# CamilleChallier/Contrastive-Masked-UNet

Hardware: AMD Instinct MI355X
Metric: pretrain images/sec/node at 512x512 (CM-UNet masked-reconstruction step) (higher is better)
Workload: dtype f16; 1 GPU; cmunet_masked_recon_unet64x5_512x512_bs32_mask0.6; optimizer=AdamW(fused), amp=dynamic loss scale (device-side GradScaler protocol), global_batch=32, parallelism=dp1

## Files before the change

### cmunet_amd/_lib.py

```python
import ctypes
import os
import subprocess

_HERE = os.path.dirname(os.path.abspath(__file__))
CSRC = os.path.join(_HERE, "csrc")
LIB_PATH = os.environ.get("CMU_LIB_PATH") or os.path.join(CSRC, "libcmunet_hip.so")

F32, F16, BF16 = 0, 1, 2

_P = ctypes.c_void_p
_I = ctypes.c_int
_L = ctypes.c_int64
_F = ctypes.c_float
_U64 = ctypes.c_uint64
_D = ctypes.c_double

_SIGS = {
    "cmu_last_error": (ctypes.c_char_p, []),
    "cmu_last_kernel": (ctypes.c_char_p, []),
    "cmu_softmax2_threshold": (_I, [_P, _F, _P, _I, _I, _I, _P]),
    "cmu_conv3x3_c1_wgrad_bn": (_I, [_P, _P, _I, _P, _L, _P, _L, _P, _P, _P, _P, _P, _P, _I, _I, _I, _I, _I, _P, _P]),
    "cmu_conv3x3_c1_wgrad_bn_w": (_I, [_P, _P, _I, _P, _L, _P, _P, _P, _P, _P, _P, _P, _I, _I, _I, _I, _I, _P, _P]),
    "cmu_soft_skeleton_ws_bytes": (_L, [_L]),
    "cmu_soft_skeleton": (_I, [_P, _P, _I, _I, _I, _I, _P, _P]),
    "cmu_cldice_sums_ws_bytes": (_L, []),
    "cmu_cldice_sums": (_I, [_P, _P, _P, _P, _L, _P, _P, _P]),
    "cmu_softmax_planes": (_I, [_P, _P, _I, _I, _I, _F, _P, _P, _I, _I, _I, _I, _P]),
    "cmu_softmax_planes_bwd": (_I, [_P, _P, _I, _P, _I, _I, _I, _I, _P]),
    "cmu_soft_skeleton_save_ws_bytes": (_L, [_L, _I]),
    "cmu_soft_skeleton_save": (_I, [_P, _P, _I, _I, _I, _I, _P, _P]),
    "cmu_soft_skeleton_bwd_ws_bytes": (_L, [_L]),
    "cmu_soft_skeleton_bwd": (_I, [_P, _P, _P, _P, _P, _P, _P, _I, _I, _I, _I, _P, _P]),
    "cmu_argmax2_mask": (_I, [_P, _I, _P, _I, _I, _I, _I, _P]),
    "cmu_plane_mask": (_I, [_P, _I, _I, _I, _P, _I, _I, _I, _I, _P]),
    "cmu_contour_points_ws_bytes": (_L, [_I, _I, _I]),
    "cmu_contour_points": (_I, [_P, _P, _P, _I, _I, _I, _P, _P]),
    "cmu_lattice_nearest_ws_bytes": (_L, [_I, _I, _I]),
    "cmu_lattice_nearest": (_I, [_P, _P, _I, _P, _I, _I, _I, _P, _P]),
    "cmu_skeletonize": (_I, [_P, _P, _I, _I, _I, _P]),
    "cmu_hausdorff_finish": (_I, [_P, _P, _P, _P, _P, _P, _I, _P]),
    "cmu_radius_finish": (_I, [_P, _P, _P, _I, _P]),
    "cmu_sgd_step": (_I, [_P, _P, _P, _P, _L, _F, _F, _F, _F, _I, _L, _F, _P]),
    "cmu_sgd_step_amp": (_I, [_P, _P, _P, _P, _L, _F, _F, _F, _F, _I, _L, _F, _P, _P]),
    "cmu_lamb_block_elems": (_I, []),
    "cmu_lamb_ws_bytes": (_L, [_I, _I]),
    "cmu_resize_bicubic_ws_bytes": (_L, [_I, _I, _I, _I, _I]),
    "cmu_resize_bicubic": (_I, [_P, _I, _I, _I, _P, _P, _P, _I, _I, _P, _P]),
    "cmu_resize_bicubic_u8_ws_bytes": (_L, [_I, _I, _I, _I, _I]),
    "cmu_resize_bicubic_u8": (_I, [_P, _I, _I, _I, _P, _P, _P, _I, _I, _P, _P]),
    "cmu_resize_nearest_u8_ws_bytes": (_L, [_I, _I]),
    "cmu_resize_nearest_u8": (_I, [_P, _I, _I, _I, _P, _I, _I, _P, _P]),
    "cmu_two_view": (_I, [_P, _I, _I, _P, _P, _U64, _P, _P, _I, _P]),
    "cmu_philox_normal": (_I, [_P, _L, _U64, _U64, _P]),
    "cmu_random_patch_mask": (_I, [_P, _I, _I, _I, _I, _I, _U64, _U64, _P]),
    "cmu_skinny_gemm_ws_bytes": (_L, [_I, _I, _L]),
    "cmu_skinny_gemm_fwd": (_I, [_P, _P, _P, _P, _I, _I, _L, _P, _P]),
    "cmu_skinny_gemm_bwd_ws_bytes": (_L, [_I, _I]),
    "cmu_skinny_gemm_dgrad": (_I, [_P, _P, _P, _I, _I, _L, _P, _P]),
    "cmu_skinny_gemm_wgrad": (_I, [_P, _P, _P, _P, _I, _I, _L, _P]),
    "cmu_lamb_step": (_I, [_P, _P, _P, _P, _P, _P, _P, _P, _I, _P, _P, _I, _F, _F, _F, _F, _I, _I, _F, _I, _I, _L, _F, _P, _P]),
    "cmu_pack_desc_bytes": (_I, []),
    "cmu_pack_desc_blocks": (_L, [_I, _I, _I, _I, _I]),
    "cmu_pack_batch": (_I, [_P, _I, _L, _I, _P]),
    "cmu_version": (_I, []),
    "cmu_set_dispatch_override": (_I, [ctypes.c_char_p, _I]),
    "cmu_dispatch_knob_name": (ctypes.c_char_p, [_I]),
    "cmu_get_dispatch_knob": (_I, [ctypes.c_char_p, ctypes.POINTER(_I), ctypes.POINTER(_I)]),
    "cmu_mfma_sustained_rate": (_I, [_I, _I, _I, _I, _P, _P, _P, _P]),
    "cmu_probe_stream_reduce": (_I, [_P, _P, _P, _L, _I, _I, _P]),
    "cmu_dtype_size": (_I, [_I]),
    "cmu_pack_conv3x3_elems": (_L, [_I, _I, _I, _I]),
    "cmu_pack_conv3x3": (_I, [_P, _P, _I, _I, _I, _I, _P]),
    "cmu_pack_convT2x2_elems": (_L, [_I, _I, _I, _I]),
    "cmu_pack_convT2x2": (_I, [_P, _P, _I, _I, _I, _I, _P]),
    "cmu_conv3x3_c1_fwd": (_I, [_P, _P, _I, _P, _P, _L, _P, _I, _I, _I, _I, _I, _P]),
    "cmu_conv3x3_fwd": (_I, [_P, _L, _P, _P, _I, _P, _P, _L, _P, _I, _I, _I, _I, _I, _I, _P]),
    "cmu_conv_ntiles": (_I, [_I, _I, _I]),
    "cmu_bn_finalize_ws_bytes": (_L, [_I]),
    "cmu_bn_finalize": (_I, [_P, _I, _L, _P, _P, _P, _P, _P, _F, _F, _I, _P, _P, _P, _P, _I, _P, _P]),
    "cmu_bnrelu_maxpool_fwd": (_I, [_P, _L, _P, _P, _P, _L, _I, _I, _I, _I, _I, _P]),
    "cmu_convT2x2_fwd": (_I, [_P, _L, _P, _P, _I, _P, _P, _P, _L, _I, _I, _I, _I, _I, _I, _P]),
    "cmu_conv1x1_head_fwd": (_I, [_P, _L, _P, _P, _P, _P, _P, _I, _I, _I, _I, _I, _I, _P]),
    "cmu_apply_to_nchw": (_I, [_P, _L, _P, _P, _I, _P, _I, _I, _I, _I, _I, _P]),
    "cmu_nchw_to_nhwc": (_I, [_P, _P, _L, _I, _I, _I, _I, _I, _P]),
    "cmu_nhwc_to_nchw": (_I, [_P, _L, _P, _I, _I, _I, _I, _I, _P]),
    "cmu_bn_bwd_ws_bytes": (_L, [_I]),
    "cmu_bn_bwd_reduce": (_I, [_P, _L, _P, _L, _P, _P, _P, _P, _P, _P, _P, _I, _I, _I, _I, _I, _P, _P]),
    "cmu_bn_bwd_apply": (_I, [_P, _L, _P, _L, _P, _P, _P, _P, _P, _P, _L, _I, _I, _I, _I, _I, _P]),
    "cmu_conv3x3_wgrad_ws_bytes": (_L, [_I, _I, _I, _I, _I, _I]),
    "cmu_conv3x3_wgrad": (_I, [_P, _L, _P, _P, _I, _P, _L, _P, _I, _I, _I, _I, _I, _I, _P, _P]),
    "cmu_conv3x3_c1_wgrad_ws_bytes": (_L, [_I, _I, _I, _I]),
    "cmu_conv3x3_c1_wgrad": (_I, [_P, _P, _I, _P, _L, _P, _I, _I, _I, _I, _I, _P, _P]),
    "cmu_maxpool_bwd": (_I, [_P, _L, _P, _L, _P, _L, _P, _P, _P, _L, _P, _P, _P, _I, _I, _I, _I, _I, _P]),
    "cmu_maxpool_bwd2": (_I, [_P, _L, _P, _L, _P, _L, _P, _L, _P, _P, _P, _L, _P, _P, _P, _I, _I, _I, _I, _I, _P]),
    "cmu_maxpool_bwd_apply": (_I, [_P, _L, _P, _L, _P, _L, _P, _L, _P, _P, _P, _P, _P, _P, _L, _I, _I, _I, _I, _I, _P]),
    "cmu_bnrelu_maxpool_fwd_masked": (_I, [_P, _L, _P, _P, _P, _I, _P, _L, _I, _I, _I, _I, _I, _P]),
    "cmu_maxpool_bwd_masked": (_I, [_P, _L, _P, _L, _P, _L, _P, _P, _P, _I, _P, _L, _I, _I, _I, _I, _I, _P]),
    "cmu_bn_bwd_finalize": (_I, [_P, _L, _P, _P, _P, _I, _P]),
    "cmu_convT2x2_dgrad": (_I, [_P, _L, _P, _P, _L, _I, _I, _I, _I, _I, _I, _P]),
    "cmu_convT2x2_dgrad_bn": (_I, [_P, _L, _P, _P, _L, _P, _L, _P, _P, _P, _P, _P, _I, _I, _I, _I, _I, _I, _P]),
    "cmu_conv3x3_dgrad_bn": (_I, [_P, _L, _P, _P, _L, _P, _L, _P, _P, _P, _P, _P, _I, _I, _I, _I, _I, _I, _P]),
    "cmu_bn_bwd_finalize_tiles": (_I, [_P, _I, _L, _P, _P, _P, _I, _P, _P]),
    "cmu_convT2x2_wgrad_ws_bytes": (_L, [_I, _I, _I, _I, _I, _I]),
    "cmu_convT2x2_wgrad": (_I, [_P, _L, _P, _P, _I, _P, _L, _P, _P, _I, _I, _I, _I, _I, _I, _P, _P]),
    "cmu_conv1x1_head_bwd_ws_bytes": (_L, [_I, _I, _I, _I, _I]),
    "cmu_conv1x1_head_bn_apply": (_I, [_P, _P, _L, _P, _P, _P, _P, _P, _P, _P, _L, _I, _I, _I, _I, _I, _I, _P]),
    "cmu_conv1x1_head_bwd": (_I, [_P, _P, _L, _P, _P, _P, _P, _L, _P, _P, _P, _P, _P, _I, _I, _I, _I, _I, _I, _P, _P]),
    "cmu_masked_mse_ws_bytes": (_L, [_I, _I]),
    "cmu_masked_mse_fwd_bwd": (_I, [_P, _I, _I, _P, _P, _P, _P, _F, _P, _I, _I, _I, _P, _P]),
    "cmu_softmax_ce_dice_ws_bytes": (_L, [_I, _I, _I]),
    "cmu_softmax_ce_dice_fwd_bwd": (_I, [_P, _P, _P, _P, _F, _I, _I, _I, _P, _P]),
    "cmu_seg_stats_ws_bytes": (_L, [_I]),
    "cmu_seg_stats_fwd": (_I, [_P, _P, _I, _P, _F, _P, _I, _I, _I, _I, _P, _P]),
    "cmu_seg_stats_bwd": (_I, [_P, _P, _I, _P, _P, _P, _P, _P, _I, _I, _I, _I, _P]),
    "cmu_pointwise_loss_ws_bytes": (_L, []),
    "cmu_pointwise_loss_fwd": (_I, [_I, _P, _P, _I, _P, _P, _P, _L, _I, _L, _P, _P]),
    "cmu_pointwise_loss_bwd": (_I, [_I, _P, _P, _I, _P, _P, _P, _P, _L, _I, _L, _P]),
    "cmu_index_ce_ws_bytes": (_L, []),
    "cmu_index_ce_fwd": (_I, [_P, _P, _I, _I, _I, _P, _L, _P, _I, _I, _I, _I, _P, _P]),
    "cmu_index_ce_bwd": (_I, [_P, _P, _I, _I, _I, _P, _L, _P, _P, _I, _I, _I, _I, _P]),
    "cmu_infonce_inbatch_fwd_bwd": (_I, [_P, _P, _P, _P, _I, _I, _I, _I, _F, _F, _P]),
    "cmu_moco_ws_bytes": (_L, [_I, _I, _I]),
    "cmu_moco_infonce_enqueue": (_I, [_P, _P, _P, _I, _P, _P, _P, _P, _P, _I, _I, _I, _F, _P, _P]),
    "cmu_l2_normalize_rows": (_I, [_P, _P, _I, _I, _P]),
    "cmu_l2_normalize_rows_bwd": (_I, [_P, _P, _P, _I, _I, _P]),
    "cmu_moco_logits_assemble": (_I, [_P, _P, _P, _P, _I, _I, _I, _F, _P]),
    "cmu_moco_logits_split": (_I, [_P, _P, _I, _I, _F, _P]),
    "cmu_moco_logits_addpos": (_I, [_P, _P, _P, _I, _I, _I, _F, _P]),
    "cmu_row_cross_entropy": (_I, [_P, _P, _P, _P, _P, _P, _I, _I, _P]),
    "cmu_scale_by_device_scalar": (_I, [_P, _P, _L, _P]),
    "cmu_patchify": (_I, [_P, _P, _I, _I, _I, _I, _I, _I, _P]),
    "cmu_masked_stats_rows": (_I, []),
    "cmu_masked_channel_stats": (_I, [_P, _L, _P, _I, _I, _P, _I, _I, _I, _I, _I, _P]),
    "cmu_mask_select": (_I, [_P, _L, _P, _P, _I, _P, _I, _I, _P, _P, _L, _I, _I, _I, _I, _I, _P]),
    "cmu_bn_bwd_reduce_masked": (_I, [_P, _L, _P, _L, _P, _P, _P, _P, _P, _P, _P, _P, _I, _L, _I, _I, _I, _I, _I, _P, _P]),
    "cmu_bn_bwd_apply_masked": (_I, [_P, _L, _P, _L, _P, _P, _P, _P, _P, _P, _L, _P, _I, _I, _I, _I, _I, _I, _P]),
    "cmu_sparse_tile_list": (_I, [_P, _I, _I, _I, _I, _I, _I, _P, _P, _P]),
    "cmu_conv3x3_tiles_supported": (_I, [_I, _I, _I, _I, _I, _I]),
    "cmu_rows_channel_stats": (_I, [_P, _L, _P, _P, _P, _I, _I, _I, _I, _I, _P]),
    "cmu_bn_bwd_reduce_rows": (_I, [_P, _L, _P, _L, _P, _P, _P, _P, _P, _P, _P, _P, _P, _L, _L, _I, _I, _I, _I, _I, _P, _P]),
    "cmu_sparse_tile_lists_max": (_I, []),
    "cmu_sparse_tile_lists": (_I, [_P, _I, _I, _I, _P, _P, _P, _P, _P, _P]),
    "cmu_sparse_pixel_lists": (_I, [_P, _P, _I, _I, _I, _P, _P, _P, _P, _P]),
    "cmu_conv3x3_c1_fwd_tiles_rows": (_I, [_L]),
    "cmu_conv3x3_c1_fwd_tiles": (_I, [_P, _P, _I, _P, _P, _L, _P, _P, _P, _L, _I, _I, _I, _I, _I, _P]),
    "cmu_conv3x3_c1_wgrad_bn_tiles": (_I, [_P, _P, _I, _P, _L, _P, _L, _P, _P, _P, _P, _P, _P, _P, _P, _L, _P, _I, _I, _I, _I, _I, _P, _P]),
    "cmu_cells_supported": (_I, [_I, _I, _I, _I, _I, _I]),
    "cmu_bn_bwd_apply_cells": (_I, [_P, _L, _P, _L, _P, _P, _P, _P, _P, _P, _L, _P, _I, _I, _I, _I, _I, _I, _I, _P]),
    "cmu_mask_select_cells": (_I, [_P, _L, _P, _P, _I, _P, _I, _I, _P, _P, _L, _I, _I, _I, _I, _I, _P]),
    "cmu_maxpool_bwd_cells": (_I, [_P, _L, _P, _L, _P, _L, _P, _P, _P, _I, _P, _L, _I, _I, _I, _I, _I, _P]),
    "cmu_cells_stats_rows": (_I, []),
    "cmu_cells_channel_stats": (_I, [_P, _L, _P, _I, _P, _I, _I, _I, _I, _I, _P]),
    "cmu_bn_bwd_reduce_cells": (_I, [_P, _L, _P, _L, _P, _P, _P, _P, _P, _P, _P, _P, _I, _L, _I, _I, _I, _I, _I, _P, _P]),
    "cmu_cells_channel_sum_ws_bytes": (_L, [_I]),
    "cmu_cells_channel_sum": (_I, [_P, _L, _P, _I, _I, _P, _P, _I, _I, _I, _I, _I, _P]),
    "cmu_sparse_pixel_list_ws_bytes": (_L, [_I, _I]),
    "cmu_sparse_pixel_list": (_I, [_P, _I, _I, _I, _I, _P, _L, _P, _P, _P]),
    "cmu_conv3x3_rows_supported": (_I, [_I, _I, _I, _I, _I, _I]),
    "cmu_conv3x3_fwd_rows": (_I, [_P, _L, _P, _P, _L, _P, _P, _L, _I, _I, _I, _I, _I, _I, _P]),
    "cmu_conv3x3_fwd_tiles": (_I, [_P, _L, _P, _P, _I, _P, _P, _L, _P, _P, _I, _I, _I, _I, _I, _I, _P]),
    "cmu_conv3x3_wgrad_tile_h": (_I, [_I, _I, _I, _I, _I, _I]),
    "cmu_conv3x3_wgrad_tiles": (_I, [_P, _L, _P, _P, _I, _P, _L, _P, _P, _P, _I, _I, _I, _I, _I, _I, _I, _P, _P]),
    "cmu_spark_loss_ws_bytes": (_L, [_I, _I]),
    "cmu_spark_loss_fwd_bwd": (_I, [_P, _P, _P, _P, _P, _F, _I, _I, _I, _P, _P]),
    "cmu_gap_fwd": (_I, [_P, _L, _P, _P, _P, _I, _I, _I, _I, _I, _P]),
    "cmu_gap_bwd": (_I, [_P, _P, _L, _I, _I, _I, _I, _I, _P]),
    "cmu_ema_update": (_I, [_P, _P, _L, _F, _P]),
    "cmu_adam_step": (_I, [_P, _P, _P, _P, _P, _L, _F, _F, _F, _F, _F, _I, _L, _F, _P, _P]),
    "cmu_adam_ema_step": (_I, [_P, _P, _P, _P, _P, _L, _F, _F, _F, _F, _F, _I, _L, _F, _P, _I, _P, _P, _P, _F, _P]),
    "cmu_skinny16_gemm_ws_bytes": (_L, [_I, _I, _L]),
    "cmu_skinny16_gemm_fwd": (_I, [_P, _P, _P, _P, _I, _I, _L, _I, _P, _P]),
    "cmu_skinny16_gemm_dgrad": (_I, [_P, _P, _P, _I, _I, _L, _I, _P]),
    "cmu_skinny16_gemm_wgrad": (_I, [_P, _P, _P, _P, _I, _I, _L, _I, _P]),
    "cmu_bn1d_colsums": (_I, [_P, _P, _I, _I, _P]),
    "cmu_bn1d_relu_fwd": (_I, [_P, _P, _L, _P, _P, _P, _P, _F, _F, _I, _I, _P, _P, _P, _I, _I, _P]),
    "cmu_bn1d_bwd_colsums": (_I, [_P, _P, _P, _P, _P, _I, _P, _I, _I, _P]),
    "cmu_bn1d_relu_bwd": (_I, [_P, _P, _P, _P, _P, _P, _I, _P, _L, _P, _P, _P, _I, _I, _P]),
    "cmu_conv1x1_nchw_fwd": (_I, [_P, _L, _P, _P, _I, _P, _P, _P, _I, _I, _I, _I, _I, _I, _P]),
    "cmu_genesis_rec_bytes": (_I, []),
    "cmu_genesis_segments": (_I, [_I, _I]),
    "cmu_genesis_sample": (_I, [_P, _P, _P, _I, _I, _I, _I, _I, _D, _D, _D, _D, _D, _U64, _U64, _P]),
    "cmu_genesis_gather_shuffle": (_I, [_P, _P, _P, _P, _P, _P, _P, _I, _I, _I, _P]),
    "cmu_genesis_bezier_ws_bytes": (_L, [_I]),
    "cmu_genesis_bezier": (_I, [_P, _P, _I, _I, _I, _P, _P, _P]),
    "cmu_genesis_intensity_paint": (_I, [_P, _P, _P, _U64, _U64, _P, _I, _I, _I, _P]),
    "cmu_genesis_mae": (_I, [_P, _P, _P, _P, _P, _I, _I, _I, _P]),
    "cmu_ftaug_rec_layout": (_I, [_P, _I]),
    "cmu_ftaug_max_ksize": (_I, []),
    "cmu_ftaug_sample": (_I, [_P, _I, _I, _I, _I, _P, _I, _U64, _U64, _P]),
    "cmu_ftaug_photometric": (_I, [_P, _I, _I, _I, _P, _P, _U64, _U64, _I, _P, _I, _P]),
    "cmu_ftaug_apply": (_I, [_P, _P, _I, _I, _I, _P, _P, _U64, _U64, _I, _P, _P, _I, _P]),
    "cmu_ftaug_resize_ws_bytes": (_L, [_I, _I, _I]),
    "cmu_ftaug_resize_onehot": (_I, [_P, _P, _I, _I, _I, _P, _P, _U64, _U64, _I, _P, _I, _P, _P, _I, _I, _P, _P]),
    "cmu_mocoviews_rec_layout": (_I, [_P, _I]),
    "cmu_mocoviews_max_ksize": (_I, []),
    "cmu_mocoviews_sample": (_I, [_P, _I, _I, _I, _P, _I, _U64, _U64, _P]),
    "cmu_mocoviews_geometry": (_I, [_P, _I, _I, _I, _P, _I, _I, _I, _P, _I, _P, _P]),
    "cmu_mocoviews_max": (_I, [_P, _P, _I, _P]),
    "cmu_mocoviews_noise": (_I, [_P, _I, _I, _P, _P, _P, _U64, _U64, _P]),
    "cmu_mse_ws_bytes": (_L, []),
    "cmu_mse_fwd_bwd": (_I, [_P, _I, _P, _P, _P, _F, _P, _I, _I, _I, _P, _P]),
    "cmu_amp_state_bytes": (_I, []),
    "cmu_amp_init": (_I, [_P, _F, _P]),
    "cmu_amp_check_finite": (_I, [_P, _L, _P, _P]),
    "cmu_amp_update": (_I, [_P, _F, _F, _I, _P]),
}

EXPORTS = tuple(_SIGS.keys())


class CmuError(RuntimeError):
    pass


def build(verbose=False):
    jobs = str(min(8, os.cpu_count() or 1))
    res = subprocess.run(["make", "-C", CSRC, "-j", jobs], capture_output=not verbose, text=True)
    if res.returncode != 0:
        raise CmuError("building libcmunet_hip.so failed:\n" + (res.stdout or "") + (res.stderr or ""))
    return LIB_PATH


_lib = None


def lib():
    global _lib
    if _lib is None:
        if not os.path.exists(LIB_PATH):
            raise CmuError(f"{LIB_PATH} is missing: run `python -c 'import __graft_entry__ as g; g.build()'` "
                           "(hipcc --offload-arch=gfx950). The HIP path has no CPU fallback.")
        import torch
        l = ctypes.CDLL(LIB_PATH)
        for name, (res, args) in _SIGS.items():
            fn = getattr(l, name, None)
            if fn is None:
                continue
            fn.restype = res
            fn.argtypes = args
        _lib = l
    return _lib


def missing_symbols():
    l = lib()
    return [n for n in _SIGS if getattr(l, n, None) is None]


class EventProfiler:

    def __init__(self, gemm_only=False):
        self.records = []
        self.gemm_only = gemm_only

    def summary(self):
        import torch
        torch.cuda.synchronize()
        out = {}
        for name, e0, e1, work, _ in self.records:
            d = out.setdefault(name, {"ms": 0.0, "calls": 0, "work": 0.0})
            d["ms"] += e0.elapsed_time(e1)
            d["calls"] += 1
            d["work"] += work
        return out

    def by_kernel(self):
        import torch
        torch.cuda.synchronize()
        out = {}
        for name, e0, e1, work, tag in self.records:
            if work <= 0 or not tag:
                continue
            d = out.setdefault(tag, {"ms": 0.0, "calls": 0, "work": 0.0, "entries": set()})
            d["ms"] += e0.elapsed_time(e1)
            d["calls"] += 1
            d["work"] += work
            d["entries"].add(name)
        return out


PROFILER = None


class DevPtr(ctypes.c_void_p):
    """A device pointer that remembers which GPU owns it (``dev``): ``call`` binds the launch to that device."""


class _StreamOfArgs:
    """Placeholder for "the current stream of the device that owns this call's tensors" (resolved inside ``call``)."""


STREAM = _StreamOfArgs()


def devptr(addr, dev):
    p = DevPtr(addr)
    p.dev = dev
    return p


def call(name, *args, work=0.0):
    l = lib()
    fn = getattr(l, name, None)
    if fn is None:
        raise CmuError(f"{name} is not exported by {LIB_PATH}")
    import torch
    dev, si = None, -1
    for i, a in enumerate(args):
        if type(a) is DevPtr:
            if dev is None:
                dev = a.dev
            elif a.dev != dev:
                raise CmuError(f"{name}: tensors on different devices (cuda:{dev} and cuda:{a.dev})")
        elif a is STREAM:
            si = i
    cur = torch.cuda.current_device()
    if dev is None:
        dev = cur
    if si >= 0:
        args = list(args)
        args[si] = ctypes.c_void_p(torch.cuda.current_stream(dev).cuda_stream)
    if dev != cur:
        with torch.cuda.device(dev):
            return _call_bound(l, fn, name, args, work)
    return _call_bound(l, fn, name, args, work)


def _call_bound(l, fn, name, args, work):
    if PROFILER is not None and (work > 0 or not PROFILER.gemm_only):
        import torch
        e0, e1 = torch.cuda.Event(enable_timing=True), torch.cuda.Event(enable_timing=True)
        e0.record()
        rc = fn(*args)
        e1.record()
        PROFILER.records.append((name, e0, e1, work, l.cmu_last_kernel().decode() if work > 0 else ""))
    else:
        rc = fn(*args)
    if rc != 0:
        raise CmuError(f"{name} failed ({rc}): {l.cmu_last_error().decode()}")
    return rc
```

### cmunet_amd/csrc/conv_igemm.hip

```cpp
#include "common.h"
#include <stdlib.h>

enum { MODE_CONV3 = 0, MODE_CONVT_FWD = 1, MODE_CONVT_DGRAD = 2 };

struct IGParams {
    const void* x;
    int64_t ldx;
    const float* in_scale;
    const float* in_shift;
    int relu_from;
    const void* w;
    int npad;
    void* y;
    int64_t ldy;
    float* stats;
    const float* bias;
    int B, H, W;
    int K;
    int N;
    int Cq;
    int nslices;
    int nslices32;
    int tilesX, tilesY, nblk;
    int64_t total_blocks;
    const void* bx;
    int64_t ldbx;
    const float *b_scale, *b_shift, *b_mean, *b_invstd;
    float* bstats;
    int buf_ok;
    unsigned fd_nblk[2], fd_tx[2], fd_ty[2];
    const int* tile_list;
    const int* tile_count;
};
static inline void cmu_fastdiv_init(unsigned d, unsigned* out) {
    unsigned s = 0;
    while ((1ull << s) < d) ++s;
    out[0] = (unsigned)((((1ull << s) - d) << 32) / d + 1);
    out[1] = s;
}

template <class TR, int MODE>
struct IGCfg {
    typedef typename TR::elem_t elem_t;
    static constexpr bool C3 = (MODE == MODE_CONV3);
    static constexpr int TAPS = C3 ? 9 : 2;
    static constexpr int HALO = C3 ? 1 : 0;
    static constexpr int LW = CMU_TW + 2 * HALO;
    static constexpr int LH = CMU_TH + 2 * HALO;
    static constexpr int NPIX = LW * LH;
    static constexpr int SLICES_A = C3 ? 1 : TAPS;
    static constexpr int PS_A = SLICES_A * 64 + 16;
    static constexpr int A_BYTES = NPIX * PS_A;
    static constexpr int PS_W = 80;
    static constexpr int BN = 64;
    static constexpr int W_BYTES = TAPS * BN * PS_W;
    static constexpr int KC = 64 / (int)sizeof(elem_t);
    static constexpr int EPC = TR::EPC;
    static constexpr int EPI_ROW = BN * (int)sizeof(elem_t) + 16;
    static constexpr int EPI_STAGE = 4 * 64 * EPI_ROW;
    static constexpr int EPI_BYTES = EPI_STAGE + 4 * BN * 2 * 4;
    static constexpr int MAIN_BYTES = A_BYTES + W_BYTES;
    static constexpr int LDS_BYTES = MAIN_BYTES > EPI_BYTES ? MAIN_BYTES : EPI_BYTES;
    static constexpr int A_CHUNKS = NPIX * SLICES_A * 4;
    static constexpr int A_ITERS = (A_CHUNKS + 255) / 256;
    static constexpr int W_CHUNKS = TAPS * BN * 4;
    static constexpr int W_ITERS = (W_CHUNKS + 255) / 256;
};

__device__ static inline int pm_row(int r) { return __builtin_popcount(r >> 2) & 1; }
__device__ static inline int pm_col(int r) { return 4 * (r >> 3) + (r & 3); }

#ifdef CMU_IG_STAMPS
__device__ unsigned long long g_ig_stamps[64 * 16 * 8];
extern "C" int cmu_debug_ig_stamps(unsigned long long* host) {
    return (int)hipMemcpyFromSymbol(host, HIP_SYMBOL(g_ig_stamps), sizeof(g_ig_stamps));
}
#define IG_STAMP(k)                                                                          \
    do {                                                                                      \
        if (stamp_slot >= 0 && s < 16 && tid == 0)                                            \
            g_ig_stamps[(stamp_slot * 16 + s) * 8 + (k)] = __builtin_amdgcn_s_memtime();      \
    } while (0)
#else
#define IG_STAMP(k) do {} while (0)
#endif

template <class TR, int MODE>
__global__ __launch_bounds__(256, 2) void conv_igemm_kernel(const IGParams p) {
    typedef IGCfg<TR, MODE> C;
    typedef typename TR::elem_t elem_t;
    extern __shared__ __attribute__((aligned(16))) unsigned char smem[];

    const int tid = threadIdx.x;
    const int lane = tid & 63;
    const int wave = tid >> 6;
    const int r = lane & 31;
    const int h = lane >> 5;

    int64_t bid = blockIdx.x;
    {
        const int64_t nb = p.total_blocks;
        const int64_t q = nb >> 3, rem = nb & 7;
        const int64_t xcd = bid & 7, local = bid >> 3;
        bid = (xcd < rem ? xcd * (q + 1) : rem * (q + 1) + (xcd - rem) * q) + local;
    }
    const int nbk = (int)(bid % p.nblk);
    const int64_t tile = bid / p.nblk;
    const int tx = (int)(tile % p.tilesX);
    const int ty = (int)((tile / p.tilesX) % p.tilesY);
    const int b = (int)(tile / ((int64_t)p.tilesX * p.tilesY));
    const int ty0 = ty * CMU_TH, tx0 = tx * CMU_TW;
    const int n0 = nbk * C::BN;

    const int Hin = (MODE == MODE_CONVT_DGRAD) ? 2 * p.H : p.H;
    const int Win = (MODE == MODE_CONVT_DGRAD) ? 2 * p.W : p.W;
    const unsigned char* xb = reinterpret_cast<const unsigned char*>(p.x);
// ... 164 lines not shown
#pragma unroll
        for (int it = 0; it < C::W_ITERS; ++it) {
            if (it * 256 + tid < C::W_CHUNKS) *reinterpret_cast<u32x4*>(smem + w_lds[it]) = wreg[it];
        }
    };

    f32x16 acc[2][2];
#pragma unroll
    for (int i = 0; i < 2; ++i)
#pragma unroll
        for (int j = 0; j < 2; ++j)
#pragma unroll
            for (int e = 0; e < 16; ++e) acc[i][j][e] = 0.f;

    int a_base[2];
#pragma unroll
    for (int i = 0; i < 2; ++i) a_base[i] = ((4 * wave + 2 * i + pm_row(r)) * C::LW + pm_col(r)) * C::PS_A + h * 16;
    const int w_base = C::A_BYTES + r * C::PS_W + h * 16;

    const int nstages = C::C3 ? p.nslices : (p.nslices + C::TAPS - 1) / C::TAPS;

#ifdef CMU_IG_STAMPS
    const int stamp_slot = (blockIdx.x % 61 == 0 && blockIdx.x / 61 < 64) ? (int)(blockIdx.x / 61) : -1;
#endif
    load_stage(0);
    for (int s = 0; s < nstages; ++s) {
        IG_STAMP(0);
        __syncthreads();
        IG_STAMP(1);
        store_stage();
        IG_STAMP(2);
        __syncthreads();
        IG_STAMP(3);
        if (s + 1 < nstages) load_stage(s + 1);
        IG_STAMP(4);
#pragma unroll
        for (int t = 0; t < C::TAPS; ++t) {
            const int aoff = C::C3 ? ((t / 3) * C::LW + (t % 3)) * C::PS_A : t * 64;
#pragma unroll
            for (int ks = 0; ks < 2; ++ks) {
                const u32x4 a0 = *reinterpret_cast<const u32x4*>(smem + a_base[0] + aoff + ks * 32);
                const u32x4 a1 = *reinterpret_cast<const u32x4*>(smem + a_base[1] + aoff + ks * 32);
                const u32x4 b0 = *reinterpret_cast<const u32x4*>(smem + w_base + (t * C::BN) * C::PS_W + ks * 32);
                const u32x4 b1 = *reinterpret_cast<const u32x4*>(smem + w_base + (t * C::BN + 32) * C::PS_W + ks * 32);
                TR::mma16(a0, b0, acc[0][0]);
                TR::mma16(a0, b1, acc[0][1]);
                TR::mma16(a1, b0, acc[1][0]);
                TR::mma16(a1, b1, acc[1][1]);
            }
        }
        IG_STAMP(5);
    }
    __syncthreads();

    float* stat_lds = reinterpret_cast<float*>(smem + C::EPI_STAGE);
    if (MODE == MODE_CONV3 && p.stats != nullptr) {
        float s1[2] = {0.f, 0.f}, s2[2] = {0.f, 0.f};
#pragma unroll
        for (int i = 0; i < 2; ++i)
#pragma unroll
            for (int e = 0; e < 16; ++e) {
                const int m32 = (e & 3) + 8 * (e >> 2) + 4 * h;
                const int row = 4 * wave + 2 * i + pm_row(m32), col = pm_col(m32);
                const bool ok = (ty0 + row < p.H) && (tx0 + col < p.W);
#pragma unroll
                for (int j = 0; j < 2; ++j) {
                    const float v = ok ? acc[i][j][e] : 0.f;
                    s1[j] += v;
                    s2[j] = fmaf(v, v, s2[j]);
                }
            }
#pragma unroll
        for (int j = 0; j < 2; ++j) {
            s1[j] += __shfl_xor(s1[j], 32, 64);
            s2[j] += __shfl_xor(s2[j], 32, 64);
            if (h == 0) {
                stat_lds[(wave * C::BN + 32 * j + r) * 2 + 0] = s1[j];
                stat_lds[(wave * C::BN + 32 * j + r) * 2 + 1] = s2[j];
            }
        }
    }
    constexpr int CPRp = C::BN / C::EPC;
    u32x4 xr[CPRp];
    if ((MODE != MODE_CONVT_FWD) && p.bstats != nullptr) {
#pragma unroll
        for (int it = 0; it < CPRp; ++it) {
            const int idx = it * 64 + lane;
            const int m = idx / CPRp, q = idx % CPRp;
            const int row = 4 * wave + 2 * (m >> 5) + pm_row(m & 31), col = pm_col(m & 31);
            const int gy = ty0 + row < p.H ? ty0 + row : p.H - 1, gx = tx0 + col < p.W ? tx0 + col : p.W - 1;
            int n = n0 + q * C::EPC;
            n = n < p.N ? n : 0;
            const int64_t xo = (((int64_t)b * p.H + gy) * p.W + gx) * p.ldbx + n;
            xr[it] = ld_global16(reinterpret_cast<const unsigned char*>(p.bx) + xo * (int64_t)sizeof(elem_t));
        }
    }
    unsigned char* my = smem + wave * (64 * C::EPI_ROW);
#pragma unroll
    for (int i = 0; i < 2; ++i)
#pragma unroll
        for (int j = 0; j < 2; ++j) {
            float badd = 0.f;
            if (MODE == MODE_CONVT_FWD) {
                const int n = n0 + 32 * j + r;
                if (n < p.N) badd = p.bias[n % p.Cq];
            }
#pragma unroll
            for (int e = 0; e < 16; ++e) {
                const int m = 32 * i + (e & 3) + 8 * (e >> 2) + 4 * h;
                *reinterpret_cast<elem_t*>(my + m * C::EPI_ROW + (32 * j + r) * (int)sizeof(elem_t)) =
                    TR::from_float(acc[i][j][e] + badd);
            }
        }
    __syncthreads();
    if (MODE == MODE_CONV3 && p.stats != nullptr && tid < C::BN) {
        const int n = n0 + tid;
        if (n < p.N) {
            float a = 0.f, q = 0.f;
#pragma unroll
            for (int w4 = 0; w4 < 4; ++w4) {
                a += stat_lds[(w4 * C::BN + tid) * 2 + 0];
                q += stat_lds[(w4 * C::BN + tid) * 2 + 1];
            }
            p.stats[(tile * 2 + 0) * p.N + n] = a;
            p.stats[(tile * 2 + 1) * p.N + n] = q;
        }
    }
    constexpr int CPR = C::BN / C::EPC;
    unsigned char* yb = reinterpret_cast<unsigned char*>(p.y);
    const bool bs = (MODE != MODE_CONVT_FWD) && p.bstats != nullptr;
    constexpr int EPCc = C::EPC;
    float bsc[EPCc], bsh[EPCc], bmu[EPCc], bis[EPCc], bs1[EPCc], bs2[EPCc];
    const int nq = n0 + (lane % CPR) * EPCc;
    if (bs) {
#pragma unroll
        for (int e = 0; e < EPCc; ++e) {
            const int c = nq + e < p.N ? nq + e : 0;
            bsc[e] = p.b_scale[c]; bsh[e] = p.b_shift[c]; bmu[e] = p.b_mean[c]; bis[e] = p.b_invstd[c];
            bs1[e] = bs2[e] = 0.f;
        }
    }
#pragma unroll
    for (int it = 0; it < (64 * CPR) / 64; ++it) {
        const int idx = it * 64 + lane;
        const int m = idx / CPR, q = idx % CPR;
        const int row = 4 * wave + 2 * (m >> 5) + pm_row(m & 31), col = pm_col(m & 31);
        const int gy = ty0 + row, gx = tx0 + col;
        const int n = n0 + q * C::EPC;
        if (gy < p.H && gx < p.W && n < p.N) {
            const u32x4 v = *reinterpret_cast<const u32x4*>(my + m * C::EPI_ROW + q * 16);
            int64_t off;
            if (MODE == MODE_CONVT_FWD) {
                const int ij = n / p.Cq, co = n % p.Cq;
                off = (((int64_t)b * (2 * p.H) + 2 * gy + (ij >> 1)) * (2 * p.W) + 2 * gx + (ij & 1)) * p.ldy + co;
            } else {
                off = (((int64_t)b * p.H + gy) * p.W + gx) * p.ldy + n;
            }
            st_global16(yb + off * (int64_t)sizeof(elem_t), v);
            if (bs) {
                float gv[EPCc], xv[EPCc];
                TR::unpack(v, gv);
                TR::unpack(xr[it], xv);
#pragma unroll
                for (int e = 0; e < EPCc; ++e) {
                    const float dz = fmaf(xv[e], bsc[e], bsh[e]) > 0.f ? gv[e] : 0.f;
                    bs1[e] += dz;
                    bs2[e] = fmaf(dz, xv[e], bs2[e]);
                }
            }
        }
    }
    if (bs) {
#pragma unroll
        for (int e = 0; e < EPCc; ++e) {
#pragma unroll
            for (int o = CPR; o < 64; o <<= 1) {
                bs1[e] += __shfl_xor(bs1[e], o, 64);
                bs2[e] += __shfl_xor(bs2[e], o, 64);
            }
            bs2[e] = (bs2[e] - bmu[e] * bs1[e]) * bis[e];
            if (lane < CPR) {
                stat_lds[(wave * C::BN + lane * EPCc + e) * 2 + 0] = bs1[e];
                stat_lds[(wave * C::BN + lane * EPCc + e) * 2 + 1] = bs2[e];
            }
        }
        __syncthreads();
        if (tid < C::BN && n0 + tid < p.N) {
            float a = 0.f, q = 0.f;
#pragma unroll
            for (int w4 = 0; w4 < 4; ++w4) {
                a += stat_lds[(w4 * C::BN + tid) * 2 + 0];
                q += stat_lds[(w4 * C::BN + tid) * 2 + 1];
            }
            p.bstats[(tile * 2 + 0) * p.N + n0 + tid] = a;
            p.bstats[(tile * 2 + 1) * p.N + n0 + tid] = q;
        }
    }
}

#include "conv_igemm3.inc"
#include "conv_igemm3p.inc"
#include "conv_igemm5.inc"
#include "conv_igemm6.inc"
#include "conv_gemm.inc"
#include "conv_gather.inc"

template <class TR, int MODE>
static int launch_igemm(const IGParams& p, hipStream_t st, const char* name) {
    typedef IGCfg<TR, MODE> C;
    static CmuPerDevice attr_set;
    if (!attr_set.done()) {
        hipError_t e = hipFuncSetAttribute(reinterpret_cast<const void*>(&conv_igemm_kernel<TR, MODE>),
                                           hipFuncAttributeMaxDynamicSharedMemorySize, C::LDS_BYTES);
        if (e != hipSuccess) {
            cmu_set_error("%s: hipFuncSetAttribute(%d B LDS): %s", name, C::LDS_BYTES, hipGetErrorString(e));
            return CMU_ERR_LAUNCH;
        }
        attr_set.mark();
    }
    hipLaunchKernelGGL((conv_igemm_kernel<TR, MODE>), dim3((unsigned)p.total_blocks), dim3(256), C::LDS_BYTES, st, p);
    cmu_set_kernel_tag("conv_igemm_kernel");
    CMU_CHECK_LAUNCH(name);
    return CMU_OK;
}

static int check_act(const char* name, const void* ptr, int64_t ld, int C, int dt) {
    const int epc = 16 / cmu_dtype_size(dt);
    CMU_CHECK_ARG(ptr != nullptr, "%s: null tensor", name);
    CMU_CHECK_ARG(cmu_aligned16(ptr), "%s: tensor not 16-byte aligned", name);
    CMU_CHECK_ARG(ld >= C && ld % epc == 0, "%s: pixel stride %lld must be >= C=%d and a multiple of %d", name, (long long)ld, C, epc);
    CMU_CHECK_ARG(C % epc == 0, "%s: channels %d must be a multiple of %d", name, C, epc);
    return CMU_OK;
}

template <class TR>
static int conv3x3_fwd_t(IGParams p, hipStream_t st) {
    typedef IGCfg<TR, MODE_CONV3> C;
    if (igemm3_eligible<TR>(p)) return launch_igemm3_any<TR>(p, st);
    p.nslices = cmu_div_up(p.K, C::KC);
    p.nslices32 = cmu_div_up(p.K, C::KC / 2);
    p.npad = cmu_conv3x3_npad(p.N);
    p.buf_ok = cmu_knob(CMU_KNOB_CONV_BUFLOAD) && ((int64_t)p.H * p.W * p.ldx + p.K) * (int64_t)sizeof(typename TR::elem_t) < 0x7fff0000ll &&
               (int64_t)p.nslices32 * 9 * p.npad * 32 < 0x7fff0000ll;
    return launch_igemm<TR, MODE_CONV3>(p, st, "cmu_conv3x3_fwd");
}
template <class TR>
static int convT_fwd_t(IGParams p, hipStream_t st) {
    typedef IGCfg<TR, MODE_CONVT_FWD> C;
    if (conv_gemm_s_eligible<TR>(p, false))
        return p.in_scale ? launch_conv_gemm_s<TR, false, true>(p, st, "cmu_convT2x2_fwd") : launch_conv_gemm_s<TR, false, false>(p, st, "cmu_convT2x2_fwd");
    if (conv_gemm_eligible<TR>(p, false))
        return p.in_scale ? launch_conv_gemm<TR, false, true>(p, st, "cmu_convT2x2_fwd") : launch_conv_gemm<TR, false, false>(p, st, "cmu_convT2x2_fwd");
    p.nslices = cmu_div_up(p.K, C::KC);
    return launch_igemm<TR, MODE_CONVT_FWD>(p, st, "cmu_convT2x2_fwd");
}
template <class TR>
static int convT_dgrad_t(IGParams p, hipStream_t st) {
    typedef IGCfg<TR, MODE_CONVT_DGRAD> C;
    {
        IGParams q = p;
        q.K = 4 * p.K;
        if (conv_gemm_s_eligible<TR>(q, true)) return launch_conv_gemm_s<TR, true, false>(q, st, "cmu_convT2x2_dgrad");
        if (conv_gemm_eligible<TR>(q, true)) return launch_conv_gemm<TR, true, false>(q, st, "cmu_convT2x2_dgrad");
    }
    p.nslices = 4 * cmu_div_up(p.K, C::KC);
    return launch_igemm<TR, MODE_CONVT_DGRAD>(p, st, "cmu_convT2x2_dgrad");
}

static void fill_tiles(IGParams& p) {
    p.tilesX = cmu_div_up(p.W, CMU_TW);
    p.tilesY = cmu_div_up(p.H, CMU_TH);
    p.nblk = cmu_div_up(p.N, 64);
    p.npad = p.nblk * 64;
    p.total_blocks = (int64_t)p.B * p.tilesX * p.tilesY * p.nblk;
}

extern "C" int cmu_conv_ntiles(int B, int H, int W) { return B * cmu_div_up(H, CMU_TH) * cmu_div_up(W, CMU_TW); }

// ... 257 lines not shown
    hipLaunchKernelGGL(sparse_tile_lists_kernel, dim3(n), dim3(1024), 0, (hipStream_t)stream, active, q);
    CMU_CHECK_LAUNCH("cmu_sparse_tile_lists");
    return CMU_OK;
}
struct SpRowsBatch {
    int f;
    int s[SP_MAX_LISTS], H[SP_MAX_LISTS];
    int* rows[SP_MAX_LISTS];
    int* count[SP_MAX_LISTS];
    long long cap[SP_MAX_LISTS];
};
__global__ void sparse_pixel_rows_multi_kernel(const int* __restrict__ plist, const int* __restrict__ pcount, SpRowsBatch q) {
    const int i = blockIdx.y;
    const int np = pcount[0], s = q.s[i], H = q.H[i], f = q.f;
    const long long n = (long long)np * s * s, cap = q.cap[i];
    int* __restrict__ rows = q.rows[i];
    for (long long r = (long long)blockIdx.x * blockDim.x + threadIdx.x; r < cap; r += (long long)gridDim.x * blockDim.x) {
        int v = -1;
        if (r < n) {
            const int pi = (int)(r / (s * s)), in = (int)(r % (s * s));
            const int t = plist[pi];
            const int fx = t % f, fy = (t / f) % f, b = t / (f * f);
            v = (b * H + fy * s + in / s) * H + fx * s + in % s;
        }
        rows[r] = v;
    }
    if (blockIdx.x == 0 && threadIdx.x == 0) q.count[i][0] = (int)(n < cap ? n : cap);
}
extern "C" int cmu_sparse_pixel_lists(const int* patches, const int* patch_count, int f, int B, int n, const int* H, int* const* rows,
                                      const int64_t* capacity, int* const* counts, void* stream) {
    CMU_CHECK_ARG(patches && patch_count && f > 0 && B > 0 && n > 0 && n <= SP_MAX_LISTS && H && rows && capacity && counts,
                  "cmu_sparse_pixel_lists: bad args (at most %d levels per call)", SP_MAX_LISTS);
    SpRowsBatch q = {};
    q.f = f;
    int64_t cmax = 0;
    for (int i = 0; i < n; ++i) {
        const int sb = sp_shift_bits(H[i], f);
        CMU_CHECK_ARG(rows[i] && counts[i] && capacity[i] > 0 && sb >= 0 && (int64_t)B * H[i] * H[i] < (1ll << 31),
                      "cmu_sparse_pixel_lists: null list, or H must be f << s (entry %d: H=%d, f=%d)", i, H[i], f);
        q.s[i] = 1 << sb; q.H[i] = H[i]; q.rows[i] = rows[i]; q.count[i] = counts[i]; q.cap[i] = capacity[i];
        if (capacity[i] > cmax) cmax = capacity[i];
    }
    const int grid = (int)(cmu_div_up64(cmax, 256) < 4096 ? cmu_div_up64(cmax, 256) : 4096);
    hipLaunchKernelGGL(sparse_pixel_rows_multi_kernel, dim3(grid, n), dim3(256), 0, (hipStream_t)stream, patches, patch_count, q);
    CMU_CHECK_LAUNCH("cmu_sparse_pixel_lists");
    return CMU_OK;
}
extern "C" int cmu_sparse_tile_list(const uint8_t* active, int f, int B, int H, int W, int tile_h, int tile_w, int* list, int* count,
                                    void* stream) {
    CMU_CHECK_ARG(active && list && count && f > 0 && B > 0 && H > 0 && W > 0 && tile_h > 0 && tile_w > 0, "cmu_sparse_tile_list: bad args");
    const int sbits = sp_shift_bits(H, f);
    CMU_CHECK_ARG(sbits >= 0 && W == H, "cmu_sparse_tile_list: H must be f << s and the level square (H=%d, W=%d, f=%d)", H, W, f);
    const int tilesY = cmu_div_up(H, tile_h), tilesX = cmu_div_up(W, tile_w);
    CMU_CHECK_ARG((int64_t)B * tilesY * tilesX < (1ll << 30), "cmu_sparse_tile_list: too many tiles");
    hipLaunchKernelGGL(sparse_tile_list_kernel, dim3(1), dim3(1024), 0, (hipStream_t)stream, active, f, sbits, B, tilesY, tilesX, tile_h, tile_w,
                       list, count);
    CMU_CHECK_LAUNCH("cmu_sparse_tile_list");
    return CMU_OK;
}

static int check_bnstats(const char* name, const void* yraw, int64_t ldy, const float* scale, const float* shift, const float* mean,
                         const float* invstd, const float* bstats, int N, int dt) {
    int rc;
    if ((rc = check_act(name, yraw, ldy, N, dt))) return rc;
    CMU_CHECK_ARG(scale && shift && mean && invstd && bstats, "%s: null BatchNorm argument", name);
    return CMU_OK;
}

extern "C" int cmu_conv3x3_dgrad_bn(const void* dY, int64_t ldd, const void* wpacked_flip, void* dX, int64_t ldx, const void* yraw,
                                    int64_t ldy, const float* scale, const float* shift, const float* save_mean,
                                    const float* save_invstd, float* bstats, int B, int H, int W, int K, int N, int dt, void* stream) {
    CMU_CHECK_ARG(B > 0 && H > 0 && W > 0 && K > 0 && N > 0, "cmu_conv3x3_dgrad_bn: bad dims");
    CMU_CHECK_ARG(cmu_dtype_size(dt) > 0, "cmu_conv3x3_dgrad_bn: bad dtype %d", dt);
    int rc;
    if ((rc = check_act("cmu_conv3x3_dgrad_bn(dY)", dY, ldd, K, dt))) return rc;
    if ((rc = check_act("cmu_conv3x3_dgrad_bn(dX)", dX, ldx, N, dt))) return rc;
    if ((rc = check_bnstats("cmu_conv3x3_dgrad_bn(yraw)", yraw, ldy, scale, shift, save_mean, save_invstd, bstats, N, dt))) return rc;
    CMU_CHECK_ARG(wpacked_flip && cmu_aligned16(wpacked_flip), "cmu_conv3x3_dgrad_bn: packed weights null/unaligned");
    CMU_CHECK_ARG((int64_t)B * cmu_div_up(H, CMU_TH) * cmu_div_up(W, CMU_TW) * cmu_div_up(N, 64) < (1ll << 31), "cmu_conv3x3_dgrad_bn: grid too large");
    IGParams p = {};
    p.x = dY; p.ldx = ldd; p.w = wpacked_flip; p.y = dX; p.ldy = ldx;
    p.B = B; p.H = H; p.W = W; p.K = K; p.N = N; p.Cq = N;
    p.bx = yraw; p.ldbx = ldy; p.b_scale = scale; p.b_shift = shift; p.b_mean = save_mean; p.b_invstd = save_invstd; p.bstats = bstats;
    fill_tiles(p);
    CMU_DISPATCH_DT(dt, conv3x3_fwd_t, p, (hipStream_t)stream);
}

extern "C" int cmu_convT2x2_dgrad_bn(const void* dOut, int64_t ldd, const void* wpacked_dgrad, void* dX, int64_t ldx, const void* yraw,
                                     int64_t ldy, const float* scale, const float* shift, const float* save_mean,
                                     const float* save_invstd, float* bstats, int B, int H, int W, int Cin, int Cout, int dt,
                                     void* stream) {
    CMU_CHECK_ARG(B > 0 && H > 0 && W > 0 && Cin > 0 && Cout > 0, "cmu_convT2x2_dgrad_bn: bad dims");
    CMU_CHECK_ARG(cmu_dtype_size(dt) > 0, "cmu_convT2x2_dgrad_bn: bad dtype %d", dt);
    int rc;
    if ((rc = check_act("cmu_convT2x2_dgrad_bn(dOut)", dOut, ldd, Cout, dt))) return rc;
    if ((rc = check_act("cmu_convT2x2_dgrad_bn(dX)", dX, ldx, Cin, dt))) return rc;
    if ((rc = check_bnstats("cmu_convT2x2_dgrad_bn(yraw)", yraw, ldy, scale, shift, save_mean, save_invstd, bstats, Cin, dt))) return rc;
    CMU_CHECK_ARG(wpacked_dgrad && cmu_aligned16(wpacked_dgrad), "cmu_convT2x2_dgrad_bn: packed weights null/unaligned");
    IGParams p = {};
    p.x = dOut; p.ldx = ldd; p.w = wpacked_dgrad; p.y = dX; p.ldy = ldx;
    p.B = B; p.H = H; p.W = W; p.K = Cout; p.N = Cin; p.Cq = Cout;
    p.bx = yraw; p.ldbx = ldy; p.b_scale = scale; p.b_shift = shift; p.b_mean = save_mean; p.b_invstd = save_invstd; p.bstats = bstats;
    fill_tiles(p);
    CMU_DISPATCH_DT(dt, convT_dgrad_t, p, (hipStream_t)stream);
}
```

### cmunet_amd/csrc/conv_igemm3.inc

```
#include <type_traits>

template <class TR, int NB_, int TWB_ = 2, int THB_ = 1>
struct IG3Cfg {
    typedef typename TR::elem_t elem_t;
    static constexpr int ES = (int)sizeof(elem_t);
    static constexpr int EPC = TR::EPC;
    static constexpr int KC = 32 / ES;
    static constexpr int NB = NB_;
    static constexpr int TWB = TWB_;
    static constexpr int THB = THB_;
    static constexpr int TH = 16 * THB, TW = 16 * TWB;
    static constexpr int LW = TW + 2, LH = TH + 2, NPIX = LW * LH;
    static constexpr int PS = 48;
    static constexpr int A_BYTES = NPIX * PS;
    static constexpr int PSB = 32;
    static constexpr int B_TAP = NB * PSB;
    static constexpr int B_BYTES = 9 * B_TAP;
    static constexpr int BUF_BYTES = A_BYTES + B_BYTES;
    static constexpr int MAIN_BYTES = 2 * BUF_BYTES;
    static constexpr int WN = NB / 64, WM = 8 / WN;
    static constexpr int RB = WM / TWB;
    static constexpr int SW = TH / 2 / RB;
    static constexpr int A_CHUNKS = NPIX * 2, A_ITERS = (A_CHUNKS + 511) / 512;
    static constexpr int B_CHUNKS = 9 * NB * 2, B_ITERS = (B_CHUNKS + 511) / 512;
    static constexpr int MAX_K = THB == 1 ? 1024 : 128;
    static constexpr int TAB_BYTES = 2 * MAX_K * 4;
    static constexpr int NFP = ES == 2 ? 2 : 1;
    static constexpr int EPI_ROW = NFP * 32 * ES + 16;
    static constexpr int EPI_WAVE = SW * 32 * EPI_ROW;
    static constexpr int EPI_STAGE = 8 * EPI_WAVE;
    static constexpr int EPI_BYTES = EPI_STAGE + 8 * 64 * 2 * 4;
#ifdef CMU_IG_STAMPS
    static constexpr int STAMP_OFF = MAIN_BYTES + TAB_BYTES;
    static constexpr int LDS_BYTES = (STAMP_OFF + 2048 > EPI_BYTES ? STAMP_OFF + 2048 : EPI_BYTES);
#else
    static constexpr int LDS_BYTES = MAIN_BYTES + TAB_BYTES > EPI_BYTES ? MAIN_BYTES + TAB_BYTES : EPI_BYTES;
#endif
    static constexpr unsigned OOB = 0x7fff0000u;
};

__device__ static inline u32x4 ig3_bload(__amdgpu_buffer_rsrc_t r, unsigned voff, unsigned soff) {
    return __builtin_bit_cast(u32x4, __builtin_amdgcn_raw_buffer_load_b128(r, (int)voff, (int)soff, 0));
}

typedef __attribute__((ext_vector_type(2))) float f32x2;
template <int SW, class OK>
__device__ __forceinline__ void ig3_lane_stats(const f32x16 (&acc)[SW][2], OK ok, float (&s1)[2], float (&s2)[2]) {
    f32x2 a[2], q[2];
#pragma unroll
    for (int j = 0; j < 2; ++j) a[j] = q[j] = f32x2{0.f, 0.f};
#pragma unroll
    for (int i = 0; i < SW; ++i)
#pragma unroll
        for (int e = 0; e < 16; e += 2) {
            const bool ok0 = ok(i, e), ok1 = ok(i, e + 1);
#pragma unroll
            for (int j = 0; j < 2; ++j) {
                const f32x2 v = {ok0 ? acc[i][j][e] : 0.f, ok1 ? acc[i][j][e + 1] : 0.f};
                a[j] += v;
                q[j] = __builtin_elementwise_fma(v, v, q[j]);
            }
        }
#pragma unroll
    for (int j = 0; j < 2; ++j) {
        s1[j] = a[j][0] + a[j][1];
        s2[j] = q[j][0] + q[j][1];
    }
}

template <int EPC>
__device__ __forceinline__ void ig3_bst_consts(const float* scale, const float* shift, int n, float (&gs)[EPC], float (&gh)[EPC]) {
#pragma unroll
    for (int e = 0; e < EPC; ++e) {
        gs[e] = scale[n + e] * 0x1p60f;
        gh[e] = shift[n + e] * 0x1p60f;
    }
}
template <class TR>
__device__ __forceinline__ void ig3_bst_accum(const u32x4& g, const u32x4& x, const float (&gs)[TR::EPC], const float (&gh)[TR::EPC],
                                              float (&bs1)[TR::EPC], float (&bs2)[TR::EPC]) {
    float gv[TR::EPC], xv[TR::EPC];
    TR::unpack(g, gv);
    TR::unpack(x, xv);
#pragma unroll
    for (int e = 0; e < TR::EPC; e += 2) {
        const float gate0 = __builtin_amdgcn_fmed3f(fmaf(xv[e], gs[e], gh[e]), 0.f, 1.f);
        const float gate1 = __builtin_amdgcn_fmed3f(fmaf(xv[e + 1], gs[e + 1], gh[e + 1]), 0.f, 1.f);
        const f32x2 dz = f32x2{gate0, gate1} * f32x2{gv[e], gv[e + 1]};
        const f32x2 s1 = f32x2{bs1[e], bs1[e + 1]} + dz;
        const f32x2 s2 = __builtin_elementwise_fma(dz, f32x2{xv[e], xv[e + 1]}, f32x2{bs2[e], bs2[e + 1]});
        bs1[e] = s1[0]; bs1[e + 1] = s1[1];
        bs2[e] = s2[0]; bs2[e + 1] = s2[1];
    }
}
template <int EPC>
__device__ __forceinline__ void ig3_bst_fold(float (&bs1)[EPC], float (&bs2)[EPC], int lane, const float* mean, const float* invstd, float* stat) {
    constexpr int H1 = EPC / 2, H2 = EPC / 4;
    float a1[H1], a2[H1], b1[H2], b2[H2];
    auto fold32 = [](float d, float s) {
        const auto r = __builtin_amdgcn_permlane32_swap(__float_as_uint(d), __float_as_uint(s), false, false);
        return __uint_as_float(r[0]) + __uint_as_float(r[1]);
    };
    auto fold16 = [](float d, float s) {
        const auto r = __builtin_amdgcn_permlane16_swap(__float_as_uint(d), __float_as_uint(s), false, false);
        return __uint_as_float(r[0]) + __uint_as_float(r[1]);
    };
    auto fold8 = [](float v) { return v + __uint_as_float(__builtin_amdgcn_update_dpp(0u, __float_as_uint(v), 0x128 , 0xf, 0xf, false)); };
#pragma unroll
    for (int e = 0; e < H1; ++e) { a1[e] = fold32(bs1[e], bs1[e + H1]); a2[e] = fold32(bs2[e], bs2[e + H1]); }
#pragma unroll
    for (int e = 0; e < H2; ++e) { b1[e] = fold8(fold16(a1[e], a1[e + H2])); b2[e] = fold8(fold16(a2[e], a2[e + H2])); }
    const int c0 = (lane & 7) * EPC + H1 * (lane >> 5) + H2 * ((lane >> 4) & 1);
    if (!(lane & 8)) {
#pragma unroll
        for (int e = 0; e < H2; ++e) {
            stat[(c0 + e) * 2 + 0] = b1[e];
            stat[(c0 + e) * 2 + 1] = (b2[e] - mean[c0 + e] * b1[e]) * invstd[c0 + e];
        }
    }
}

template <class TR, int NB, int TWB>
__device__ __forceinline__ void ig3_epilogue(const IGParams& p, unsigned char* smem, f32x16 (&acc)[IG3Cfg<TR, NB, TWB>::SW][2], int tid, int lane,
                                             int wave, int wn, int wrow, int wcol, int r, int h, int b, int ty, int tx, int ty0, int tx0,
                                             int n0) {
    typedef IG3Cfg<TR, NB, TWB> C;
    typedef typename TR::elem_t elem_t;
    constexpr int EPC = TR::EPC;
    constexpr int SW = C::SW;
    float* stat_lds = reinterpret_cast<float*>(smem + C::EPI_STAGE);
    const int row0 = wrow * 2 * SW, col0 = wcol * 16;
    if (p.stats != nullptr) {
        float s1[2], s2[2];
        ig3_lane_stats<SW>(acc, [&](int i, int e) {
            const int m32 = (e & 3) + 8 * (e >> 2) + 4 * h;
            const int row = row0 + 2 * i + pm_row(m32), col = col0 + pm_col(m32);
            return (ty0 + row < p.H) && (tx0 + col < p.W);
        }, s1, s2);
#pragma unroll
        for (int j = 0; j < 2; ++j) {
            s1[j] += __shfl_xor(s1[j], 32, 64);
            s2[j] += __shfl_xor(s2[j], 32, 64);
            if (h == 0) {
                stat_lds[(wave * 64 + 32 * j + r) * 2 + 0] = s1[j];
                stat_lds[(wave * 64 + 32 * j + r) * 2 + 1] = s2[j];
            }
        }
    }
    unsigned char* my = smem + wave * C::EPI_WAVE;
    unsigned char* yb = reinterpret_cast<unsigned char*>(p.y);
    constexpr int CPR = C::NFP * 32 / EPC;
    auto write_slab = [&](float* dst) {
        if (tid < TWB * NB) {
            const int half = tid / NB, c = tid % NB;
            const int tx16 = TWB * tx + half, tiles16 = (p.W + 15) / 16;
            if (tx16 < tiles16 && n0 + c < p.N) {
                float a = 0.f, q = 0.f;
#pragma unroll
                for (int wr = 0; wr < C::RB; ++wr) {
                    const int wv = (c / 64) * C::WM + wr * TWB + half;
                    a += stat_lds[(wv * 64 + (c & 63)) * 2 + 0];
                    q += stat_lds[(wv * 64 + (c & 63)) * 2 + 1];
                }
                const int64_t t16 = ((int64_t)b * p.tilesY + ty) * tiles16 + tx16;
                dst[(t16 * 2 + 0) * p.N + n0 + c] = a;
                dst[(t16 * 2 + 1) * p.N + n0 + c] = q;
            }
        }
    };
    constexpr int NIT = (SW * 32 * CPR) / 64;
    float badd[2] = {0.f, 0.f};
    const bool cq64 = p.bias != nullptr && (p.Cq & 63) == 0;
    int ij_w = 0, co_w = 0;
    if (p.bias != nullptr) {
        const int nw = n0 + wn * 64;
        ij_w = nw / p.Cq;
        co_w = nw - ij_w * p.Cq;
#pragma unroll
        for (int j = 0; j < 2; ++j) badd[j] = p.bias[cq64 ? co_w + 32 * j + r : (nw + 32 * j + r) % p.Cq];
    }
#pragma unroll
    for (int jp = 0; jp < 2 / C::NFP; ++jp) {
        if (jp > 0) __syncthreads();
        u32x4 xr[NIT];
        if (p.bstats != nullptr) {
#pragma unroll
            for (int it = 0; it < NIT; ++it) {
                const int idx = it * 64 + lane;
                const int m = idx / CPR, q = idx % CPR;
                const int row = row0 + 2 * (m >> 5) + pm_row(m & 31), col = col0 + pm_col(m & 31);
                const int gy = ty0 + row < p.H ? ty0 + row : p.H - 1, gx = tx0 + col < p.W ? tx0 + col : p.W - 1;
                const int n = n0 + wn * 64 + jp * C::NFP * 32 + q * EPC;
                const int64_t pixel = ((int64_t)b * p.H + gy) * p.W + gx;
                xr[it] = ld_global16(reinterpret_cast<const unsigned char*>(p.bx) + (pixel * p.ldbx + n) * (int64_t)sizeof(elem_t));
            }
        }
#pragma unroll
        for (int i = 0; i < SW; ++i)
#pragma unroll
            for (int jj = 0; jj < C::NFP; ++jj)
#pragma unroll
                for (int e = 0; e < 16; ++e) {
                    const int m = 32 * i + (e & 3) + 8 * (e >> 2) + 4 * h;
                    *reinterpret_cast<elem_t*>(my + m * C::EPI_ROW + (32 * jj + r) * C::ES) =
                        TR::from_float(acc[i][jp * C::NFP + jj][e] + badd[jp * C::NFP + jj]);
                }
        __syncthreads();
        if (jp == 0 && p.stats != nullptr) write_slab(p.stats);
        float bsc[EPC], bsh[EPC], bs1[EPC], bs2[EPC];
        const int nq = n0 + wn * 64 + jp * C::NFP * 32 + (lane % CPR) * EPC;
        if (p.bstats != nullptr) {
            ig3_bst_consts<EPC>(p.b_scale, p.b_shift, nq, bsc, bsh);
#pragma unroll
            for (int e = 0; e < EPC; ++e) bs1[e] = bs2[e] = 0.f;
        }
#pragma unroll
        for (int it = 0; it < NIT; ++it) {
            const int idx = it * 64 + lane;
            const int m = idx / CPR, q = idx % CPR;
            const int row = row0 + 2 * (m >> 5) + pm_row(m & 31), col = col0 + pm_col(m & 31);
            const int gy = ty0 + row, gx = tx0 + col;
            const int n = n0 + wn * 64 + jp * C::NFP * 32 + q * EPC;
            if (gy < p.H && gx < p.W) {
                const u32x4 v = *reinterpret_cast<const u32x4*>(my + m * C::EPI_ROW + q * 16);
                const int64_t pixel = ((int64_t)b * p.H + gy) * p.W + gx;
                if (p.bias != nullptr) {
                    const int ij = cq64 ? ij_w : n / p.Cq, co = cq64 ? co_w + (n - (n0 + wn * 64)) : n % p.Cq;
                    const int64_t po = ((int64_t)b * (2 * p.H) + 2 * gy + (ij >> 1)) * (2 * p.W) + 2 * gx + (ij & 1);
                    st_global16_nt(yb + (po * p.ldy + co) * (int64_t)sizeof(elem_t), v);
                } else {
                    st_global16_nt(yb + (pixel * p.ldy + n) * (int64_t)sizeof(elem_t), v);
                }
                if (p.bstats != nullptr) ig3_bst_accum<TR>(v, xr[it], bsc, bsh, bs1, bs2);
            }
        }
        if (p.bstats != nullptr) {
            const int nb0 = n0 + wn * 64 + jp * C::NFP * 32;
            ig3_bst_fold<EPC>(bs1, bs2, lane, p.b_mean + nb0, p.b_invstd + nb0, stat_lds + (wave * 64 + jp * C::NFP * 32) * 2);
        }
    }
    if (p.bstats != nullptr) {
        __syncthreads();
        write_slab(p.bstats);
    }
}

template <class TR, int NB, bool TF, int TWB>
__global__ __launch_bounds__(512) void conv_igemm3_kernel(const IGParams p) {
    typedef IG3Cfg<TR, NB, TWB> C;
    constexpr int EPC = TR::EPC;
    constexpr int SW = C::SW;
    extern __shared__ __attribute__((aligned(16))) unsigned char smem[];

    const int tid = threadIdx.x;
    const int lane = tid & 63;
    const int wave = __builtin_amdgcn_readfirstlane(tid >> 6);
    const int r = lane & 31;
    const int h = lane >> 5;
    const int wm = wave % C::WM, wn = wave / C::WM;
    const int wcol = wm % TWB, wrow = wm / TWB;

    int64_t bid = blockIdx.x;
    {
        const int64_t nb = p.total_blocks;
        const int64_t q = nb >> 3, rem = nb & 7;
        const int64_t xcd = bid & 7, local = bid >> 3;
        bid = (xcd < rem ? xcd * (q + 1) : rem * (q + 1) + (xcd - rem) * q) + local;
    }
    const int nbk = (int)(bid % p.nblk);
    const int64_t tile = bid / p.nblk;
    const int tx = (int)(tile % p.tilesX);
    const int ty = (int)((tile / p.tilesX) % p.tilesY);
    const int b = (int)(tile / ((int64_t)p.tilesX * p.tilesY));
    const int ty0 = ty * C::TH, tx0 = tx * C::TW;
    const int n0 = nbk * NB;

    const int64_t img_elems = (int64_t)p.H * p.W * p.ldx;
    const unsigned char* ximg = reinterpret_cast<const unsigned char*>(p.x) + (int64_t)b * img_elems * C::ES;
    const unsigned x_bytes = (unsigned)((((int64_t)p.H * p.W - 1) * p.ldx + p.K) * C::ES);
    const __amdgpu_buffer_rsrc_t rs_x = __builtin_amdgcn_make_buffer_rsrc(const_cast<unsigned char*>(ximg), 0, (int)x_bytes, 0x00020000);
    const unsigned w_bytes = (unsigned)((int64_t)p.nslices32 * 9 * p.npad * 32);
    const __amdgpu_buffer_rsrc_t rs_w = __builtin_amdgcn_make_buffer_rsrc(const_cast<void*>(p.w), 0, (int)w_bytes, 0x00020000);

    const int cg = tid & 1;
    unsigned a_voff[C::A_ITERS];
    unsigned a_inb = 0;
#pragma unroll
    for (int it = 0; it < C::A_ITERS; ++it) {
        const int pix = it * 256 + (tid >> 1);
        const int py = pix / C::LW, px = pix % C::LW;
        const int gy = ty0 - 1 + py, gx = tx0 - 1 + px;
        const bool ok = pix < C::NPIX && gy >= 0 && gy < p.H && gx >= 0 && gx < p.W;
        a_voff[it] = ok ? (unsigned)((((int64_t)gy * p.W + gx) * p.ldx + cg * EPC) * C::ES) : C::OOB;
        a_inb |= (ok ? 1u : 0u) << it;
    }
    const bool a_last_live = ((C::A_ITERS - 1) * 256 + (tid >> 1)) < C::NPIX;
    const unsigned a_st = (unsigned)((tid >> 1) * C::PS + cg * 16);
    unsigned b_voff[C::B_ITERS];
#pragma unroll
    for (int it = 0; it < C::B_ITERS; ++it) {
        const int row = it * 256 + (tid >> 1);
        const int t = row / NB, n = row % NB;
        b_voff[it] = row < 9 * NB ? (unsigned)(((int64_t)t * p.npad + n0 + n) * 32 + cg * 16) : C::OOB;
    }
    const bool b_last_live = ((C::B_ITERS - 1) * 256 + (tid >> 1)) < 9 * NB;
    const unsigned b_st = (unsigned)(C::A_BYTES + (tid >> 1) * C::PSB + ((cg ^ ((tid >> 4) & 1)) * 16));
    const unsigned w_slice = (unsigned)p.npad * 32u * 9u;

    u32x4 areg[C::A_ITERS], breg[C::B_ITERS];
    const int nsl = p.nslices32;
    float* tab = reinterpret_cast<float*>(smem + C::MAIN_BYTES);
    if (TF)
        for (int c = tid; c < p.K; c += 512) {
            tab[c] = p.in_scale[c];
            tab[C::MAX_K + c] = p.in_shift[c];
        }
    auto issue_loads = [&](int s) {
#pragma unroll
        for (int it = 0; it < C::A_ITERS; ++it) areg[it] = ig3_bload(rs_x, a_voff[it], (unsigned)(s * 32));
#pragma unroll
        for (int it = 0; it < C::B_ITERS; ++it) breg[it] = ig3_bload(rs_w, b_voff[it], (unsigned)s * w_slice);
    };
    auto store_regs = [&](unsigned buf, int s) {
        float sc[EPC], sh[EPC];
        float lo = 0.f;
        if (TF) {
// ... 221 lines not shown
```

### cmunet_amd/csrc/conv_igemm3p.inc

```

template <class TR, int NB, int THB = 1, bool WRES = false>
struct IG3PCfg {
    typedef IG3Cfg<TR, NB, 2, THB> C;
    static constexpr int WRES_SLICES = 4;
    static constexpr int A_STRIDE = WRES ? C::A_BYTES : C::BUF_BYTES;
    static constexpr int B_BASE = WRES ? 2 * C::A_BYTES : C::A_BYTES;
    static constexpr int MAIN_BYTES = WRES ? 2 * C::A_BYTES + WRES_SLICES * C::B_BYTES : C::MAIN_BYTES;
    static constexpr int STAT_OFF = MAIN_BYTES + C::TAB_BYTES;
    static constexpr int STAT_BYTES = 8 * 64 * 2 * 4;
    static constexpr int EPI_OFF = STAT_OFF + STAT_BYTES;
    static constexpr int EPI_WAVE1 = 16 * C::EPI_ROW;
#ifdef CMU_IG_STAMPS
    static constexpr int STAMP_OFF = MAIN_BYTES + 1024;
    static constexpr int STAMP_ITERS = 12;
    static constexpr int LDS_BYTES = EPI_OFF + 8 * EPI_WAVE1;
#else
    static constexpr int LDS_BYTES = EPI_OFF + 8 * EPI_WAVE1;
#endif
};

template <class TR, int NB, bool TF, bool BST, int THB = 1, bool WRES = false, bool PART = false>
__global__ __launch_bounds__(512) void conv_igemm3p_kernel(const IGParams p) {
    typedef IG3Cfg<TR, NB, 2, THB> C;
    typedef IG3PCfg<TR, NB, THB, WRES> P;
// ... 483 lines not shown
            s_regs = s_ld;
            inb_regs = a_inb;
        }
#ifndef CMU_IG_STAMPS_EPI
        IG3P_STAMP(5);
#endif
        if (++s_mma == nsl) {
            s_mma = 0;
            ++i_mma;
        }
        if (!second) __syncthreads();
#ifndef CMU_IG_STAMPS_EPI
        IG3P_STAMP(6);
#endif
    }
    __syncthreads();
#ifdef CMU_IG_STAMPS
    if (stamp_slot >= 0 && tid < 2 * P::STAMP_ITERS * 8) g_ig_stamps[stamp_slot * 256 + tid] = stamp_lds[tid];
    if (stamp_slot >= 0 && tid == 0) {
        g_ig_stamps[stamp_slot * 256 + 200] = __builtin_amdgcn_s_memtime() - clk0;
        g_ig_stamps[stamp_slot * 256 + 201] = __builtin_amdgcn_s_memrealtime() - rt0;
        g_ig_stamps[stamp_slot * 256 + 202] = (unsigned long long)G;
    }
#endif
    write_slab(decode(n_my - 1));
}

static int cmu_num_cus() {
    static int n[256] = {0};
    const int dev = cmu_current_device() & 255;
    int v = __atomic_load_n(&n[dev], __ATOMIC_RELAXED);
    if (v == 0) {
        int cus = 0;
        if (hipDeviceGetAttribute(&cus, hipDeviceAttributeMultiprocessorCount, dev) != hipSuccess || cus <= 0) cus = 256;
        v = cus;
        __atomic_store_n(&n[dev], v, __ATOMIC_RELAXED);
    }
    return v;
}

template <class TR, int NB, bool TF, bool BST, int THB = 1, bool WRES = false, bool PART = false>
static int launch_igemm3p_cfg(IGParams p, hipStream_t st) {
    typedef IG3Cfg<TR, NB, 2, THB> C;
    typedef IG3PCfg<TR, NB, THB, WRES> P;
    static_assert(P::LDS_BYTES <= 163840, "LDS budget");
    static CmuPerDevice attr_set;
    if (!attr_set.done()) {
        hipError_t e = hipFuncSetAttribute(reinterpret_cast<const void*>(&conv_igemm3p_kernel<TR, NB, TF, BST, THB, WRES, PART>),
                                           hipFuncAttributeMaxDynamicSharedMemorySize, P::LDS_BYTES);
        if (e != hipSuccess) {
            cmu_set_error("cmu_conv3x3_fwd(wide, persistent): hipFuncSetAttribute(%d B LDS): %s", P::LDS_BYTES, hipGetErrorString(e));
            return CMU_ERR_LAUNCH;
        }
        attr_set.mark();
    }
    p.tilesX = cmu_div_up(p.W, C::TW);
    p.tilesY = cmu_div_up(p.H, C::TH);
    p.nblk = p.N / NB;
    p.nslices32 = p.K / C::KC;
    p.nslices = p.nslices32;
    p.npad = cmu_conv3x3_npad(p.N);
    p.total_blocks = (int64_t)p.B * p.tilesX * p.tilesY * p.nblk;
    if (p.total_blocks >= (1ll << 30)) return launch_igemm3_cfg<TR, NB, TF, 2>(p, st);
    cmu_fastdiv_init((unsigned)p.nblk, p.fd_nblk);
    cmu_fastdiv_init((unsigned)p.tilesX, p.fd_tx);
    cmu_fastdiv_init((unsigned)p.tilesY, p.fd_ty);
    const int forced = cmu_knob(CMU_KNOB_CONV_PERSIST_GRID);
    const int64_t want = forced > 0 ? forced : cmu_num_cus();
    const int64_t grid = p.total_blocks < want ? p.total_blocks : want;
    hipLaunchKernelGGL((conv_igemm3p_kernel<TR, NB, TF, BST, THB, WRES, PART>), dim3((unsigned)grid), dim3(512), P::LDS_BYTES, st, p);
    cmu_set_kernel_tag("conv_igemm3p_kernel");
    CMU_CHECK_LAUNCH("cmu_conv3x3_fwd(wide, persistent)");
    return CMU_OK;
}

static bool cmu_conv_persist_enabled() { return cmu_knob(CMU_KNOB_CONV_PERSIST); }
template <class TR> static bool igemm5_eligible(const IGParams& p);
template <class TR> static int launch_igemm5(const IGParams& p, hipStream_t st);
template <class TR> static bool igemm6_eligible(const IGParams& p);
template <class TR> static int launch_igemm6(const IGParams& p, hipStream_t st);
template <class TR>
static int launch_igemm3_any(const IGParams& p, hipStream_t st) {
    if (!cmu_conv_persist_enabled()) return launch_igemm3<TR>(p, st);
    if (igemm6_eligible<TR>(p)) return launch_igemm6<TR>(p, st);
    if (igemm5_eligible<TR>(p)) return launch_igemm5<TR>(p, st);
    const bool tf = p.in_scale != nullptr, bst = p.bstats != nullptr;
    if (tf && bst) return launch_igemm3<TR>(p, st);
    if (p.K / (32 / (int)sizeof(typename TR::elem_t)) < 4) return launch_igemm3<TR>(p, st);
    if (p.H % 16 != 0 || p.W % 32 != 0) {
        if (!igemm3_persist_part_enabled() || igemm3_slim_tiles(p, (int)sizeof(typename TR::elem_t))) return launch_igemm3<TR>(p, st);
        if (p.N % 128 == 0 && !igemm3_narrow_blocks(p))
            return tf ? launch_igemm3p_cfg<TR, 128, true, false, 1, false, true>(p, st)
                      : (bst ? launch_igemm3p_cfg<TR, 128, false, true, 1, false, true>(p, st) : launch_igemm3p_cfg<TR, 128, false, false, 1, false, true>(p, st));
        return tf ? launch_igemm3p_cfg<TR, 64, true, false, 1, false, true>(p, st)
                  : (bst ? launch_igemm3p_cfg<TR, 64, false, true, 1, false, true>(p, st) : launch_igemm3p_cfg<TR, 64, false, false, 1, false, true>(p, st));
    }
    if (p.N % 128 == 0 && !igemm3_narrow_blocks(p))
        return tf ? launch_igemm3p_cfg<TR, 128, true, false>(p, st)
                  : (bst ? launch_igemm3p_cfg<TR, 128, false, true>(p, st) : launch_igemm3p_cfg<TR, 128, false, false>(p, st));
    if constexpr (sizeof(typename TR::elem_t) == 2) {
        if (cmu_knob(CMU_KNOB_CONV_WRES) && p.N == 64 && p.K == 64)
            return tf ? launch_igemm3p_cfg<TR, 64, true, false, 1, true>(p, st)
                      : (bst ? launch_igemm3p_cfg<TR, 64, false, true, 1, true>(p, st) : launch_igemm3p_cfg<TR, 64, false, false, 1, true>(p, st));
    }
    return tf ? launch_igemm3p_cfg<TR, 64, true, false>(p, st)
              : (bst ? launch_igemm3p_cfg<TR, 64, false, true>(p, st) : launch_igemm3p_cfg<TR, 64, false, false>(p, st));
}
```

### cmunet_amd/csrc/elementwise.hip

```cpp
#include "common.h"
#include <string.h>

static thread_local char g_err[512] = "";
void cmu_set_error(const char* fmt, ...) {
    va_list ap;
    va_start(ap, fmt);
    vsnprintf(g_err, sizeof(g_err), fmt, ap);
    va_end(ap);
}
extern "C" const char* cmu_last_error(void) { return g_err; }
static thread_local const char* g_kernel_tag = "";
void cmu_set_kernel_tag(const char* tag) { g_kernel_tag = tag; }
extern "C" const char* cmu_last_kernel(void) { return g_kernel_tag; }
extern "C" int cmu_version(void) { return 100; }

#define CMU_KNOB_UNREAD INT32_MIN
struct CmuKnobRow {
    const char* name;
    int kind, dflt, floor;
    int env = CMU_KNOB_UNREAD, ovr = -1;
};
#define CMU_KNOB_ROW(id, kind, dflt, floor) {"CMU_" #id, CMU_KNOB_##kind, dflt, floor},
static CmuKnobRow g_knobs[CMU_KNOB_COUNT] = {CMU_KNOBS(CMU_KNOB_ROW)};
int cmu_knob(int id) {
// ... 527 lines not shown
    CMU_DISPATCH_DT(dt, conv3x3_c1_fwd_t, x, mask, mask_per_sample, w, y, ldy, stats, B, H, W, Cout, (hipStream_t)stream);
}

extern "C" int cmu_conv3x3_c1_fwd_tiles_rows(int64_t max_tiles) { return (int)(max_tiles < CMU_C1F_CAP ? (max_tiles < 1 ? 1 : max_tiles) : CMU_C1F_CAP); }
extern "C" int cmu_conv3x3_c1_fwd_tiles(const float* x, const uint8_t* mask, int mask_per_sample, const float* w, void* y, int64_t ldy,
                                        float* stats, const int* tile_list, const int* tile_count, int64_t max_tiles, int B, int H, int W,
                                        int Cout, int dt, void* stream) {
    const int es = cmu_dtype_size(dt);
    CMU_CHECK_ARG(es > 0, "cmu_conv3x3_c1_fwd_tiles: bad dtype");
    const int epc = 16 / es;
    CMU_CHECK_ARG(x && w && y && tile_list && tile_count && B > 0 && H > 0 && W > 0, "cmu_conv3x3_c1_fwd_tiles: bad args");
    CMU_CHECK_ARG(Cout % epc == 0 && Cout / epc <= 256 && Cout > 0, "cmu_conv3x3_c1_fwd_tiles: Cout=%d must be a multiple of %d (<= %d)", Cout, epc, 256 * epc);
    CMU_CHECK_ARG(cmu_aligned16(y) && ldy % epc == 0 && ldy >= Cout, "cmu_conv3x3_c1_fwd_tiles: y alignment / stride");
    if (max_tiles < 1) max_tiles = 1;
    CMU_DISPATCH_DT(dt, conv3x3_c1_fwd_t, x, mask, mask_per_sample, w, y, ldy, stats, B, H, W, Cout, (hipStream_t)stream, tile_list, tile_count,
                    max_tiles);
}

template <class TR>
__global__ void bnrelu_maxpool_kernel(const unsigned char* __restrict__ y, int64_t ldy, const float* __restrict__ scale,
                                      const float* __restrict__ shift, unsigned char* __restrict__ out, int64_t ldo, int B, int H,
                                      int W, int C, int64_t total, const uint8_t* __restrict__ amask = nullptr, int f = 0, int sbits = 0) {
    constexpr int EPC = TR::EPC;
    constexpr int ES = (int)sizeof(typename TR::elem_t);
    const int nchunk = C / EPC;
    const int Ho = H / 2, Wo = W / 2;
    for (int64_t o = (int64_t)blockIdx.x * blockDim.x + threadIdx.x; o < total; o += (int64_t)gridDim.x * blockDim.x) {
        int ch, xo, yo, b;
        int64_t pix;
        if (total <= 0x7fffffffll) {
            const unsigned ou = (unsigned)o, pq = ou / (unsigned)nchunk;
            ch = (int)(ou - pq * (unsigned)nchunk);
            pix = pq;
        } else {
            ch = (int)(o % nchunk);
            pix = o / nchunk;
        }
        cmu_pixel_coords(pix, Wo, Ho, total <= 0x7fffffffll, b, yo, xo);
        if (amask != nullptr && !sp_active(amask, f, sbits, b, 2 * yo, 2 * xo, 0)) {
            st_global16(out + ((((int64_t)b * Ho + yo) * Wo + xo) * ldo + ch * EPC) * ES, u32x4{0u, 0u, 0u, 0u});
            continue;
        }
        float sc[EPC], sh[EPC], m[EPC];
#pragma unroll
        for (int e = 0; e < EPC; ++e) {
            sc[e] = scale[ch * EPC + e];
            sh[e] = shift[ch * EPC + e];
            m[e] = 0.f;
        }
#pragma unroll
        for (int q = 0; q < 4; ++q) {
            const int64_t src = (((int64_t)b * H + 2 * yo + (q >> 1)) * W + 2 * xo + (q & 1)) * ldy + ch * EPC;
            float f[EPC];
            TR::unpack(ld_global16_nt(y + src * ES), f);
#pragma unroll
            for (int e = 0; e < EPC; ++e) m[e] = fmaxf(m[e], fmaf(f[e], sc[e], sh[e]));
        }
        st_global16(out + ((((int64_t)b * Ho + yo) * Wo + xo) * ldo + ch * EPC) * ES, TR::pack(m));
    }
}
template <class TR>
static int bnrelu_maxpool_t(const void* y, int64_t ldy, const float* scale, const float* shift, void* out, int64_t ldo, int B, int H,
                            int W, int C, hipStream_t st, const uint8_t* amask = nullptr, int f = 0) {
    const int64_t total = (int64_t)B * (H / 2) * (W / 2) * (C / TR::EPC);
#ifndef CMU_POOLF_CAP
#define CMU_POOLF_CAP 65536
#endif
    const int grid = (int)(cmu_div_up64(total, 256) < CMU_POOLF_CAP ? cmu_div_up64(total, 256) : CMU_POOLF_CAP);
    hipLaunchKernelGGL((bnrelu_maxpool_kernel<TR>), dim3(grid), dim3(256), 0, st, (const unsigned char*)y, ldy, scale, shift,
                       (unsigned char*)out, ldo, B, H, W, C, total, amask, f, amask ? sp_shift_bits(H, f) : 0);
    CMU_CHECK_LAUNCH("cmu_bnrelu_maxpool_fwd");
    return CMU_OK;
}
extern "C" int cmu_bnrelu_maxpool_fwd(const void* y, int64_t ldy, const float* scale, const float* shift, void* out, int64_t ldo,
                                      int B, int H, int W, int C, int dt, void* stream) {
    const int es = cmu_dtype_size(dt);
    CMU_CHECK_ARG(es > 0 && y && out && scale && shift, "cmu_bnrelu_maxpool_fwd: bad args");
    const int epc = 16 / es;
    CMU_CHECK_ARG(H % 2 == 0 && W % 2 == 0 && H > 0 && W > 0 && B > 0, "cmu_bnrelu_maxpool_fwd: H,W must be even (got %d,%d)", H, W);
    CMU_CHECK_ARG(C % epc == 0 && ldy % epc == 0 && ldo % epc == 0 && ldy >= C && ldo >= C, "cmu_bnrelu_maxpool_fwd: C/ld alignment");
    CMU_CHECK_ARG(cmu_aligned16(y) && cmu_aligned16(out), "cmu_bnrelu_maxpool_fwd: pointer alignment");
    CMU_DISPATCH_DT(dt, bnrelu_maxpool_t, y, ldy, scale, shift, out, ldo, B, H, W, C, (hipStream_t)stream);
}
extern "C" int cmu_bnrelu_maxpool_fwd_masked(const void* y, int64_t ldy, const float* scale, const float* shift, const uint8_t* active, int f,
                                             void* out, int64_t ldo, int B, int H, int W, int C, int dt, void* stream) {
    const int es = cmu_dtype_size(dt);
    CMU_CHECK_ARG(es > 0 && y && out && scale && shift && active && f > 0, "cmu_bnrelu_maxpool_fwd_masked: bad args");
    const int epc = 16 / es;
    CMU_CHECK_ARG(H % 2 == 0 && W % 2 == 0 && H > 0 && W > 0 && B > 0, "cmu_bnrelu_maxpool_fwd_masked: H,W must be even (got %d,%d)", H, W);
    CMU_CHECK_ARG(C % epc == 0 && ldy % epc == 0 && ldo % epc == 0 && ldy >= C && ldo >= C, "cmu_bnrelu_maxpool_fwd_masked: C/ld alignment");
    CMU_CHECK_ARG(cmu_aligned16(y) && cmu_aligned16(out), "cmu_bnrelu_maxpool_fwd_masked: pointer alignment");
    const int sbits = sp_shift_bits(H, f);
    CMU_CHECK_ARG(sbits >= 1 && (f << sbits) == W, "cmu_bnrelu_maxpool_fwd_masked: H=%d, W=%d must be f=%d times a power of two >= 2 (a pool window lies in one patch)", H, W, f);
    CMU_DISPATCH_DT(dt, bnrelu_maxpool_t, y, ldy, scale, shift, out, ldo, B, H, W, C, (hipStream_t)stream, active, f);
}

constexpr int HEAD_MAX_K = 8;
template <class TR, int KT>
__global__ void conv1x1_head_fwd_kernel(const unsigned char* __restrict__ x, int64_t ldx, const float* __restrict__ scale,
                                        const float* __restrict__ shift, const float* __restrict__ w, const float* __restrict__ bias,
                                        float* __restrict__ logits, int B, int H, int W, int C, int K, int64_t npix) {
    constexpr int EPC = TR::EPC;
    constexpr int ES = (int)sizeof(typename TR::elem_t);
    constexpr int U = 4;
    const int nchunk = C / EPC;
    const int ch = threadIdx.x % nchunk;
    const int ppb = blockDim.x / nchunk;
    float sc[EPC], sh[EPC], wk[KT][EPC];
#pragma unroll
    for (int e = 0; e < EPC; ++e) {
        sc[e] = scale ? scale[ch * EPC + e] : 1.f;
        sh[e] = scale ? shift[ch * EPC + e] : 0.f;
    }
#pragma unroll
    for (int k = 0; k < KT; ++k)
#pragma unroll
        for (int e = 0; e < EPC; ++e) wk[k][e] = (k < K) ? w[k * C + ch * EPC + e] : 0.f;
    const float lo = scale ? 0.f : -__builtin_inff();
    const int64_t HW = (int64_t)H * W;
    for (int64_t p0 = (int64_t)blockIdx.x * ppb * U; p0 < npix; p0 += (int64_t)gridDim.x * ppb * U) {
        u32x4 q[U];
        bool ok[U];
#pragma unroll
        for (int u = 0; u < U; ++u) {
            const int64_t pix = p0 + u * ppb + threadIdx.x / nchunk;
            ok[u] = pix < npix;
            q[u] = ok[u] ? ld_global16(x + (pix * ldx + ch * EPC) * ES) : u32x4{0u, 0u, 0u, 0u};
        }
#pragma unroll
        for (int u = 0; u < U; ++u) {
            const int64_t pix = p0 + u * ppb + threadIdx.x / nchunk;
            float f[EPC];
            TR::unpack(q[u], f);
            float acc[KT];
#pragma unroll
            for (int k = 0; k < KT; ++k) acc[k] = 0.f;
#pragma unroll
            for (int e = 0; e < EPC; ++e) {
                const float a = fmaxf(fmaf(f[e], sc[e], sh[e]), lo);
#pragma unroll
                for (int k = 0; k < KT; ++k) acc[k] = fmaf(a, wk[k][e], acc[k]);
            }
#pragma unroll
            for (int k = 0; k < KT; ++k)
                if (k < K)
                    for (int o = 1; o < nchunk; o <<= 1) acc[k] += __shfl_xor(acc[k], o, 64);
            if (ok[u] && ch == 0) {
                int64_t b, r;
                if (npix <= 0x7fffffffll) {
                    const unsigned bq = (unsigned)pix / (unsigned)HW;
                    b = bq; r = (unsigned)pix - bq * (unsigned)HW;
                } else {
                    b = pix / HW; r = pix % HW;
                }
#pragma unroll
                for (int k = 0; k < KT; ++k)
                    if (k < K) logits[(b * K + k) * HW + r] = acc[k] + bias[k];
            }
        }
    }
}
template <class TR>
static int conv1x1_head_fwd_t(const void* x, int64_t ldx, const float* scale, const float* shift, const float* w, const float* bias,
                              float* logits, int B, int H, int W, int C, int K, hipStream_t st) {
    const int nchunk = C / TR::EPC;
    const int64_t npix = (int64_t)B * H * W;
// ... 85 lines not shown
```

### cmunet_amd/engine.py

```python
import os
import weakref

import torch

from . import _lib, ops
from .ops import Act
from .optim import claim_grad_sink

BN_EPS = 1e-5
BN_MOMENTUM = 0.1


_FUSE_HEAD = os.environ.get("CMU_HEAD_FUSE", "1") != "0"
_FUSE_DGRAD_BN = os.environ.get("CMU_DGRAD_BN", "1")
_FUSE_POOL = os.environ.get("CMU_POOL_FUSE", "1") != "0"
_POISON_NEW = os.environ.get("CMU_POISON_NEW", "0") == "1"
_FUSE_POOL2 = os.environ.get("CMU_POOL_FUSE2", "1") != "0"
_C1W_RECOMP = os.environ.get("CMU_C1W_RECOMP", "1") != "0"


class _Scratch:

    def __init__(self, device):
        self.device = device
        self.bufs = {}

    def get(self, key, nbytes):
        nbytes = max(int(nbytes), 16)
        b = self.bufs.get(key)
        if b is None or b.numel() < nbytes:
            b = torch.empty(nbytes, dtype=torch.uint8, device=self.device)
            self.bufs[key] = b
        return b


class _PackCache:

    def __init__(self):
        self.items = {}

    def get(self, key, param, fn):
        ver = (param._version, ops.PARAM_GENERATION)
        hit = self.items.get(key)
        if hit is not None and hit[0] == ver and hit[1] == param.data_ptr():
            return hit[2]
        packed = fn()
        self.items[key] = (ver, param.data_ptr(), packed)
        return packed


class _Ctx(dict):
    __slots__ = ("__weakref__",)


class UNetEngine:
    def __init__(self, dt="bf16", device="cuda"):
        self.dt = ops.dt_code(dt)
        self.tdt = ops.TORCH_DT[self.dt]
        self.device = torch.device(device)
        self.scratch = _Scratch(self.device)
        self.packs = _PackCache()
        self.lib = _lib.lib()
        self._zero_pending = []
        self._cats, self._cats_busy, self._cats_owner = None, False, None
        self._nbt, self._nbt_defer = [], 0
        self.grad_target = None
        self.grad_prefix = ""

    def _gbuf(self, name, like):
        if self.grad_target is not None:
            t = self.grad_target.get(self.grad_prefix + name)
            if t is not None:
                return t
        else:
            t = claim_grad_sink(like)
            if t is not None and t.device == self.device:
                return t
        return torch.empty(like.shape, dtype=torch.float32, device=self.device)

    def _new(self, B, H, W, C):
        if _POISON_NEW:
            return Act(torch.full((B, H, W, C), float("nan"), dtype=self.tdt, device=self.device))
        return Act(torch.empty((B, H, W, C), dtype=self.tdt, device=self.device))

    def _f32(self, *shape):
        return torch.empty(shape, dtype=torch.float32, device=self.device)

    def prepack(self, sd):
        plan = getattr(self, "_pack_plan", None)
        if plan is None or plan[0] != tuple((k, v.data_ptr()) for k, v in sd.items() if k.endswith("weight") and v.dim() == 4):
            keys, items = [], []
            for k, v in sd.items():
                if not (k.endswith("weight") and v.dim() == 4):
                    continue
                name = k[:-len("weight")]
                if v.shape[2:] == (3, 3) and v.shape[1] > 1:
                    for flip in (False, True):
                        keys.append((name, flip)); items.append((v.detach(), 0, int(flip)))
                elif v.shape[2:] == (2, 2):
                    for mode in (0, 1):
                        keys.append((name, "T", mode)); items.append((v.detach(), 1, mode))
            if not items:
                return
            sig = tuple((k, v.data_ptr()) for k, v in sd.items() if k.endswith("weight") and v.dim() == 4)
            plan = (sig, keys, ops.PackPlan(items, self.dt), [sd[k[0] + "weight"] for k in keys])
            self._pack_plan = plan
        _, keys, pp, params = plan
        stamp = (ops.PARAM_GENERATION, tuple(prm._version for prm in params))
        if getattr(self, "_pack_stamp", None) == stamp and all(k in self.packs.items for k in keys):
            return
        self._pack_stamp = stamp
        pp.run()
        for key, out, prm in zip(keys, pp.outs, params):
            self.packs.items[key] = ((prm._version, ops.PARAM_GENERATION), prm.data_ptr(), out)

    def _wp(self, name, w, flip):
        return self.packs.get((name, flip), w, lambda: ops.pack_conv3x3(w.detach(), self.dt, flip))

    def _wpT(self, name, w, mode):
        return self.packs.get((name, "T", mode), w, lambda: ops.pack_convT2x2(w.detach(), self.dt, mode))

    def flush_counters(self):
        if self._nbt_defer > 0:
            return
        pend, self._nbt = self._nbt, []
        if pend:
            torch._foreach_add_(pend, 1)

    def flush_zero_bias(self):
        pend, self._zero_pending = self._zero_pending, []
        if pend:
            torch._foreach_zero_(pend)

    def _convbn_fwd(self, sd, pconv, pbn, x, out, training, x_img=None, mask=None, mask_per_sample=False, affine_out=None):
        w = sd[pconv + "weight"]
        Cout = w.shape[0]
        B, H, W = out.B, out.H, out.W
        stats = ops.new_stats(B, H, W, Cout, self.device) if training else None
        if x_img is not None:
            ops.conv3x3_c1_fwd(x_img, w.detach(), out, stats, mask, mask_per_sample)
        else:
            ops.conv3x3_fwd(x, self._wp(pconv, w, False), out, stats)
        scale, shift = affine_out if affine_out is not None else (self._f32(Cout), self._f32(Cout))
        mean, invstd = self._f32(Cout), self._f32(Cout)
        ws = self.scratch.get("bnfin", self.lib.cmu_bn_finalize_ws_bytes(Cout))
        ops.bn_finalize(stats, B * H * W, sd[pconv + "bias"].detach(), sd[pbn + "weight"].detach(),
                        sd[pbn + "bias"].detach(), sd[pbn + "running_mean"], sd[pbn + "running_var"], BN_MOMENTUM,
                        BN_EPS, training, scale, shift, mean, invstd, ws)
        if training and (pbn + "num_batches_tracked") in sd:
            self._nbt.append(sd[pbn + "num_batches_tracked"])
        return {"pconv": pconv, "pbn": pbn, "x": x, "x_img": x_img, "mask": mask, "mps": mask_per_sample,
                "y": out.with_transform(scale, shift, 0), "mean": mean, "invstd": invstd,
                "w_ver": (w._version, w.data_ptr(), ops.PARAM_GENERATION) if x_img is not None else None}

    def _double_conv_fwd(self, sd, prefix, x, out2, training, x_img=None, mask=None, mask_per_sample=False, affine_out2=None):
        w1 = sd[prefix + "0.weight"]
        B, H, W = out2.B, out2.H, out2.W
        y1 = self._new(B, H, W, w1.shape[0])
        s1 = self._convbn_fwd(sd, prefix + "0.", prefix + "1.", x, y1, training, x_img, mask, mask_per_sample)
        s2 = self._convbn_fwd(sd, prefix + "3.", prefix + "4.", s1["y"], out2, training, affine_out=affine_out2)
        self.flush_counters()
        return s1, s2

    def _bn_ws(self, C):
        return self.scratch.get("bnbwd", self.lib.cmu_bn_bwd_ws_bytes(C))

    def _tile_slab(self, y):
        n = ops.ntiles(y.B, y.H, y.W)
        return self.scratch.get("bst", n * 2 * y.C * 4)[:n * 2 * y.C * 4].view(torch.float32).view(n, 2, y.C)

    def _convbn_bwd(self, sd, s, dA, grads, need_dx, dx_out=None, fused_stats=False, next_bn=None, head=None, pool=None):
        y = s["y"]
        B, H, W, C = y.B, y.H, y.W, y.C
        w = sd[s["pconv"] + "weight"]
        dgamma, dbeta = self._gbuf(s["pbn"] + "weight", sd[s["pbn"] + "weight"]), self._gbuf(s["pbn"] + "bias", sd[s["pbn"] + "bias"])
        coef = self._f32(2, C)
        ws = self._bn_ws(C)
        bst = s.pop("bstats", None)
        if bst is not None:
            ops.bn_bwd_finalize_tiles(bst, B * H * W, dgamma, dbeta, coef,
                                      self.scratch.get("bnfin", self.lib.cmu_bn_finalize_ws_bytes(C)))
        elif fused_stats:
            ops.bn_bwd_finalize(ws, B * H * W, dgamma, dbeta, coef)
        else:
            ops.bn_bwd_reduce(dA, y, s["mean"], s["invstd"], dgamma, dbeta, coef, ws)
        first = s["x_img"] is not None
        if head is not None:
            assert dA is None and fused_stats and not first
            dY = self._new(B, H, W, C)
            ops.conv1x1_head_bn_apply(head[0], y, head[1], s["mean"], s["invstd"], coef, dY)
        elif pool is not None:
            assert dA is None and fused_stats and not first
            dY = self._new(B, H, W, C)
            ops.maxpool_bwd_apply(pool[0], pool[1], y, s["mean"], s["invstd"], coef, dY, dSkip2=pool[2])
        else:
            dY = Act(dA.buf, dA.coff, dA.C)
            if not first:
                ops.bn_bwd_apply(dA, y, s["mean"], s["invstd"], coef, dY)
        grads[s["pbn"] + "weight"] = dgamma
        grads[s["pbn"] + "bias"] = dbeta
        gb = self._gbuf(s["pconv"] + "bias", sd[s["pconv"] + "bias"])
        self._zero_pending.append(gb)
        grads[s["pconv"] + "bias"] = gb
        dW = self._gbuf(s["pconv"] + "weight", w)
        if s["x_img"] is not None:
            wsb = self.scratch.get("wg", self.lib.cmu_conv3x3_c1_wgrad_ws_bytes(B, H, W, C))
            same_w = (_C1W_RECOMP and s.get("w_ver") == (w._version, w.data_ptr(), ops.PARAM_GENERATION)
                      and getattr(self.lib, "cmu_conv3x3_c1_wgrad_bn_w", None) is not None)
            ops.conv3x3_c1_wgrad_bn(s["x_img"], dA, y, y.scale, y.shift, s["mean"], s["invstd"], coef, dW, wsb, s["mask"], s["mps"],
                                    w=w.detach() if same_w else None)
        else:
            Cin = w.shape[1]
            wsb = self.scratch.get("wg", self.lib.cmu_conv3x3_wgrad_ws_bytes(B, H, W, Cin, C, self.dt))
            ops.conv3x3_wgrad(s["x"], dY, dW, wsb)
        grads[s["pconv"] + "weight"] = dW
        if not need_dx or first:
            return None
        dX = dx_out if dx_out is not None else self._new(B, H, W, w.shape[1])
        if next_bn is not None and next_bn["y"].C == dX.C and (_FUSE_DGRAD_BN == "1" or (_FUSE_DGRAD_BN == "64" and dX.C <= 64)
                                                                or (_FUSE_DGRAD_BN == "128" and dX.C <= 128)):
            slab = self._tile_slab(next_bn["y"])
            ops.conv3x3_dgrad_bn(dY, self._wp(s["pconv"], w, True), dX, next_bn["y"], next_bn["mean"], next_bn["invstd"], slab)
            next_bn["bstats"] = slab
        else:
            ops.conv3x3_fwd(dY, self._wp(s["pconv"], w, True), dX, None)
        return dX

    @staticmethod
    def n_down(sd, prefix=""):
        n = 0
        while f"{prefix}down_conv{n + 1}.double_conv.double_conv.0.weight" in sd:
            n += 1
        return n

    def encoder_forward(self, sd, x_bhw, training, prefix="", mask=None, mask_per_sample=False, skip_out=None, skip_affine=None):
        B, H, W = x_bhw.shape
        nd = self.n_down(sd, prefix)
        assert H % (1 << nd) == 0 and W % (1 << nd) == 0, f"H,W must be multiples of {1 << nd}"
        ctx = {"levels": [], "prefix": prefix}
        self._nbt_defer += 1
        x_act, x_img = None, x_bhw.contiguous()
        h, w_ = H, W
        for i in range(1, nd + 1):
            p = f"{prefix}down_conv{i}.double_conv.double_conv."
            C = sd[p + "0.weight"].shape[0]
            out2 = skip_out[i - 1] if skip_out is not None else self._new(B, h, w_, C)
            s1, s2 = self._double_conv_fwd(sd, p, x_act, out2, training, x_img, mask if i == 1 else None, mask_per_sample,
                                           affine_out2=skip_affine[i - 1] if skip_affine is not None else None)
            pooled = self._new(B, h // 2, w_ // 2, C)
            ops.bnrelu_maxpool_fwd(s2["y"], pooled)
            ctx["levels"].append({"s1": s1, "s2": s2, "pooled": pooled})
            x_act, x_img = pooled, None
            h, w_ = h // 2, w_ // 2
        p = f"{prefix}double_conv.double_conv."
        C = sd[p + "0.weight"].shape[0]
        s1, s2 = self._double_conv_fwd(sd, p, x_act, self._new(B, h, w_, C), training, x_img, mask if nd == 0 else None, mask_per_sample)
        ctx["bott"] = {"s1": s1, "s2": s2}
        ctx["latent"] = s2["y"]
        ctx["skips"] = [lv["s2"]["y"] for lv in ctx["levels"]]
        self._nbt_defer -= 1
        self.flush_counters()
        return ctx

    def encoder_backward(self, sd, ctx, d_latent, d_skips, grads, after_bottleneck=None):
        b = ctx["bott"]
        dA = self._convbn_bwd(sd, b["s2"], d_latent, grads, True, next_bn=b["s1"])
        dP = self._convbn_bwd(sd, b["s1"], dA, grads, len(ctx["levels"]) > 0)
        if after_bottleneck is not None:
            self.flush_zero_bias()
            after_bottleneck()
        for i in range(len(ctx["levels"]), 0, -1):
            lv = ctx["levels"][i - 1]
            y2 = lv["s2"]["y"]
            ds = d_skips[i - 1] if d_skips is not None else None
            ds, ds2 = ds if isinstance(ds, (tuple, list)) else (ds, None)
            if _FUSE_POOL and (ds2 is None or _FUSE_POOL2):
                ops.maxpool_bwd(dP, ds, y2, None, lv["s2"]["mean"], lv["s2"]["invstd"], self._bn_ws(y2.C), dSkip2=ds2)
                dA1 = self._convbn_bwd(sd, lv["s2"], None, grads, True, fused_stats=True, next_bn=lv["s1"], pool=(dP, ds, ds2))
            else:
                dA2 = self._new(y2.B, y2.H, y2.W, y2.C)
                ops.maxpool_bwd(dP, ds, y2, dA2, lv["s2"]["mean"], lv["s2"]["invstd"], self._bn_ws(y2.C), dSkip2=ds2)
                dA1 = self._convbn_bwd(sd, lv["s2"], dA2, grads, True, fused_stats=True, next_bn=lv["s1"])
            dP = self._convbn_bwd(sd, lv["s1"], dA1, grads, i > 1)
        self.flush_zero_bias()
        return None

    def decoder_alloc(self, sd, B, H, W, prefix=""):
        cats = []
        i = 1
        h, w_ = H, W
        while f"{prefix}up_conv{i}.double_conv.double_conv.0.weight" in sd:
            wt = sd[f"{prefix}up_conv{i}.double_conv.double_conv.0.weight"]
            Cout, C2 = wt.shape[0], wt.shape[1]
            Cs = C2 - Cout if f"{prefix}up_conv{i}.up_sample.weight" not in sd else sd[f"{prefix}up_conv{i}.up_sample.weight"].shape[1]
            buf = self._new(B, h, w_, C2).buf
            scale = torch.ones(C2, dtype=torch.float32, device=self.device)
            shift = torch.zeros(C2, dtype=torch.float32, device=self.device)
            cats.append({"buf": buf, "scale": scale, "shift": shift, "Cup": Cs, "Cskip": C2 - Cs})
            i += 1
            h, w_ = h // 2, w_ // 2
        return cats

    def decoder_alloc_shared(self, sd, B, H, W, prefix_a, prefix_b):
        ca, cb = [], []
        i = 1
        h, w_ = H, W
        while f"{prefix_a}up_conv{i}.double_conv.double_conv.0.weight" in sd:
            wa = sd[f"{prefix_a}up_conv{i}.double_conv.double_conv.0.weight"]
            wb = sd.get(f"{prefix_b}up_conv{i}.double_conv.double_conv.0.weight")
            ka, kb = f"{prefix_a}up_conv{i}.up_sample.weight", f"{prefix_b}up_conv{i}.up_sample.weight"
            if wb is None or ka not in sd or kb not in sd:
                return None
            Cup_a, Cup_b = sd[ka].shape[1], sd[kb].shape[1]
            Cs = wa.shape[1] - Cup_a
            epc = 16 // torch.empty(0, dtype=self.tdt).element_size()
            if Cs <= 0 or wb.shape[1] - Cup_b != Cs or any(c % epc for c in (Cup_a, Cup_b, Cs)):
                return None
            C3 = Cup_a + Cs + Cup_b
            buf = self._new(B, h, w_, C3).buf
            scale = torch.ones(C3, dtype=torch.float32, device=self.device)
            shift = torch.zeros(C3, dtype=torch.float32, device=self.device)
            ca.append({"buf": buf, "scale": scale[:Cup_a + Cs], "shift": shift[:Cup_a + Cs], "Cup": Cup_a, "Cskip": Cs})
            cb.append({"buf": buf, "scale": scale[Cup_a:], "shift": shift[Cup_a:], "Cup": Cup_b, "Cskip": Cs, "base": Cup_a, "skip_first": True})
            i += 1
            h, w_ = h // 2, w_ // 2
        return ca, cb

    def rotated_weights(self, sd, prefix, cats):
        store = self.__dict__.setdefault("_rot_w", {})
        over = dict(sd)
        for i, cat in enumerate(cats, start=1):
            if not cat.get("skip_first"):
                continue
            k = f"{prefix}up_conv{i}.double_conv.double_conv.0.weight"
            w = sd[k]
            Cup = cat["Cup"]
            ent = store.get(k)
            if ent is None or ent[0].shape != w.shape or ent[0].device != w.device:
                ent = [torch.empty_like(w, dtype=torch.float32), None]
                store[k] = ent
            ver = (w._version, w.data_ptr(), ops.PARAM_GENERATION)
            if ent[1] != ver:
                torch.cat((w.detach()[:, Cup:], w.detach()[:, :Cup]), 1, out=ent[0])
                ent[1] = ver
            over[k] = ent[0]
        return over

    def unrotate_grads(self, sd, prefix, cats, grads):
        for i, cat in enumerate(cats, start=1):
            if not cat.get("skip_first"):
                continue
            k = f"{prefix}up_conv{i}.double_conv.double_conv.0.weight"
            g_rot = grads.get(k)
            if g_rot is None:
                continue
            Cs = cat["Cskip"]
            g = self._gbuf(k, sd[k])
            if g.data_ptr() == g_rot.data_ptr():
                g_rot = g_rot.clone()
            torch.cat((g_rot[:, Cs:], g_rot[:, :Cs]), 1, out=g)
            grads[k] = g

    def decoder_forward(self, sd, latent, skips, training, prefix="", cats=None, head=True):
        B = latent.B
        nup = len(skips)
        if cats is None:
            cats = self.decoder_alloc(sd, B, skips[0].H, skips[0].W, prefix)
        ctx = {"levels": [None] * nup, "prefix": prefix, "cats": cats}
        self._nbt_defer += 1
        x = latent
        for i in range(nup, 0, -1):
            p = f"{prefix}up_conv{i}."
            cat = cats[i - 1]
            Cup, Cs = cat["Cup"], cat["Cskip"]
            sk = skips[i - 1]
            assert sk.C == Cs
            base, sf = cat.get("base", 0), bool(cat.get("skip_first", False))
            up_off, sk_off = base + (Cs if sf else 0), base + (0 if sf else Cup)
            s_lo = 0 if sf else Cup
            if not (sk.buf is cat["buf"] and sk.coff == sk_off):
                cat["buf"][..., sk_off:sk_off + Cs].copy_(sk.buf[..., sk.coff:sk.coff + sk.C])
            if sk.scale is not None:
                if sk.scale.data_ptr() != cat["scale"][s_lo:].data_ptr():
                    cat["scale"][s_lo:s_lo + Cs].copy_(sk.scale)
                    cat["shift"][s_lo:s_lo + Cs].copy_(sk.shift)
                cat["ident"] = False
                relu_from = -Cs if sf else Cup
            else:
                if not cat.get("ident", False):
                    cat["scale"][s_lo:s_lo + Cs].fill_(1.0)
                    cat["shift"][s_lo:s_lo + Cs].zero_()
                    cat["ident"] = True
                relu_from = Cup + Cs
            wt = sd[p + "up_sample.weight"]
            left = Act(cat["buf"], up_off, Cup)
            ops.convT2x2_fwd(x, self._wpT(p + "up_sample.", wt, 0), sd[p + "up_sample.bias"].detach(), left)
            cat_act = Act(cat["buf"], base, Cup + Cs, cat["scale"], cat["shift"], relu_from)
            Cout = sd[p + "double_conv.double_conv.0.weight"].shape[0]
            s1, s2 = self._double_conv_fwd(sd, p + "double_conv.double_conv.", cat_act, self._new(B, sk.H, sk.W, Cout), training)
            ctx["levels"][i - 1] = {"s1": s1, "s2": s2, "x_up": x, "cat": cat}
            x = s2["y"]
        ctx["out"] = x
        if head:
            K = sd[prefix + "conv_last.weight"].shape[0]
            logits = self._f32(B, K, x.H, x.W)
            ops.conv1x1_head_fwd(x, sd[prefix + "conv_last.weight"].detach().reshape(K, -1), sd[prefix + "conv_last.bias"].detach(), logits)
            ctx["logits"] = logits
        self._nbt_defer -= 1
        self.flush_counters()
        return ctx

    def decoder_backward(self, sd, ctx, dlogits, grads, need_input_grads=True, latent_bn=None):
        prefix = ctx["prefix"]
        x = ctx["out"]
        K = sd[prefix + "conv_last.weight"].shape[0]
        wl = sd[prefix + "conv_last.weight"]
        dWl, dbl = self._gbuf(prefix + "conv_last.weight", wl), self._gbuf(prefix + "conv_last.bias", sd[prefix + "conv_last.bias"])
        ws = self.scratch.get("head", self.lib.cmu_conv1x1_head_bwd_ws_bytes(x.B, x.H, x.W, x.C, K))
        last = ctx["levels"][0]["s2"] if ctx["levels"] else None
        fused = last is not None and last["y"] is x
        dl, wl2 = dlogits.contiguous(), wl.detach().reshape(K, -1)
        head = (dl, wl2) if (fused and _FUSE_HEAD) else None
        dA = None if head is not None else self._new(x.B, x.H, x.W, x.C)
        ops.conv1x1_head_bwd(dl, x, wl2, dA, dWl.view(K, -1), dbl, ws,
                             last["mean"] if fused else None, last["invstd"] if fused else None, self._bn_ws(x.C) if fused else None)
        grads[prefix + "conv_last.weight"] = dWl
        grads[prefix + "conv_last.bias"] = dbl
        nup = len(ctx["levels"])
        d_skips = [None] * nup
        for i in range(1, nup + 1):
            lv = ctx["levels"][i - 1]
            p = f"{prefix}up_conv{i}."
            cat = lv["cat"]
            Cup, Cs = cat["Cup"], cat["Cskip"]
            dA1 = self._convbn_bwd(sd, lv["s2"], dA, grads, True, fused_stats=(fused and i == 1), next_bn=lv["s1"],
                                   head=head if i == 1 else None)
            dcat = self._convbn_bwd(sd, lv["s1"], dA1, grads, True)
            sf = bool(cat.get("skip_first", False))
            d_skips[i - 1] = Act(dcat.buf, 0 if sf else Cup, Cs)
            dleft = Act(dcat.buf, Cs if sf else 0, Cup)
            wt = sd[p + "up_sample.weight"]
            xu = lv["x_up"]
            dWt, dbt = self._gbuf(p + "up_sample.weight", wt), self._gbuf(p + "up_sample.bias", sd[p + "up_sample.bias"])
            wsb = self.scratch.get("wg", self.lib.cmu_convT2x2_wgrad_ws_bytes(xu.B, xu.H, xu.W, xu.C, Cup, self.dt))
            ops.convT2x2_wgrad(xu, dleft, dWt, dbt, wsb)
            grads[p + "up_sample.weight"] = dWt
            grads[p + "up_sample.bias"] = dbt
            if i < nup or need_input_grads:
                dA = self._new(xu.B, xu.H, xu.W, xu.C)
                tgt = ctx["levels"][i]["s2"] if i < nup else latent_bn
                if tgt is not None and tgt["y"].buf is xu.buf and tgt["y"].coff == xu.coff and tgt["y"].C == xu.C:
                    slab = self._tile_slab(tgt["y"])
                    ops.convT2x2_dgrad_bn(dleft, self._wpT(p + "up_sample.", wt, 1), dA, tgt["y"], tgt["mean"], tgt["invstd"], slab)
                    tgt["bstats"] = slab
                else:
                    ops.convT2x2_dgrad(dleft, self._wpT(p + "up_sample.", wt, 1), dA)
            else:
                dA = None
        self.flush_zero_bias()
        return dA, d_skips

    def unet_forward(self, sd, x_bhw, training, mask=None, mask_per_sample=False):
        B, H, W = x_bhw.shape
        key = (B, H, W, self.tdt)
        if self._cats_busy and (self._cats_owner is None or self._cats_owner() is None):
            self._cats_busy = False
        owns = False
        if self._cats_busy:
            cats = self.decoder_alloc(sd, B, H, W, "")
        else:
            if self._cats is None or self._cats[0] != key:
                self._cats = (key, self.decoder_alloc(sd, B, H, W, ""))
            cats = self._cats[1]
            self._cats_busy = bool(training)
            owns = True
        skip_out = [Act(c["buf"], c["Cup"], c["Cskip"]) for c in cats]
        skip_affine = [(c["scale"][c["Cup"]:], c["shift"][c["Cup"]:]) for c in cats]
        ectx = self.encoder_forward(sd, x_bhw, training, "", mask, mask_per_sample, skip_out, skip_affine)
        dctx = self.decoder_forward(sd, ectx["latent"], ectx["skips"], training, "", cats, True)
        ctx = _Ctx(enc=ectx, dec=dctx)
        if owns and training:
            self._cats_owner = weakref.ref(ctx)
        return dctx["logits"], ctx

    def unet_backward(self, sd, ctx, dlogits, after_decoder=None, after_bottleneck=None):
        grads = {}
        d_latent, d_skips = self.decoder_backward(sd, ctx["dec"], dlogits, grads, True, latent_bn=ctx["enc"]["bott"]["s2"])
        if after_decoder is not None:
            after_decoder()
        self.encoder_backward(sd, ctx["enc"], d_latent, d_skips, grads, after_bottleneck)
        if self._cats is not None and ctx["dec"]["cats"] is self._cats[1]:
            self._cats_busy = False
        return grads
```

### cmunet_amd/ops.py

```python
import ctypes
import os

import torch

from . import _lib
from ._lib import F32, F16, BF16, call

TORCH_DT = {F32: torch.float32, F16: torch.float16, BF16: torch.bfloat16}
DT_OF = {v: k for k, v in TORCH_DT.items()}
DT_NAME = {F32: "f32", F16: "f16", BF16: "bf16"}
NAME_DT = {"f32": F32, "fp32": F32, "float32": F32, "f16": F16, "fp16": F16, "float16": F16, "bf16": BF16, "bfloat16": BF16}


def dt_code(dt):
    if isinstance(dt, str):
        return NAME_DT[dt]
    if isinstance(dt, torch.dtype):
        return DT_OF[dt]
    return int(dt)


def _stream():
    return _lib.STREAM

# ... 109 lines not shown
            if kind == 0:
                Cout, Cin = w.shape[0], w.shape[1]
                n = l.cmu_pack_conv3x3_elems(Cin, Cout, dt, int(mode))
            else:
                Cin, Cout = w.shape[0], w.shape[1]
                n = l.cmu_pack_convT2x2_elems(Cin, Cout, dt, int(mode))
            out = torch.empty(n, dtype=TORCH_DT[dt], device=dev)
            self.outs.append(out)
            recs.append(struct.pack("<QQiiiiqq", w.data_ptr(), out.data_ptr(), Cin, Cout, int(mode), kind, n, block))
            block += l.cmu_pack_desc_blocks(kind, Cin, Cout, dt, int(mode))
        self.ptrs = [w.data_ptr() for w, _, _ in items]
        self.items = items
        self.total_blocks = block
        self.descs = torch.frombuffer(bytearray(b"".join(recs)), dtype=torch.uint8).to(dev)

    def run(self):
        assert all(w.data_ptr() == q for (w, _, _), q in zip(self.items, self.ptrs)), "a packed weight moved"
        call("cmu_pack_batch", _p(self.descs), len(self.items), self.total_blocks, self.dt, _stream())


def ntiles(B, H, W):
    return _lib.lib().cmu_conv_ntiles(B, H, W)


def new_stats(B, H, W, C, device):
    return torch.empty((ntiles(B, H, W), 2, C), dtype=torch.float32, device=device)


def conv3x3_c1_fwd(x_bhw, w, out, stats=None, mask=None, mask_per_sample=False):
    B, H, W = x_bhw.shape
    Cout = w.shape[0]
    assert out.C == Cout and (out.B, out.H, out.W) == (B, H, W)
    if mask is not None:
        assert mask.dtype == torch.uint8 and mask.is_contiguous()
    call("cmu_conv3x3_c1_fwd", _p(_f32c(x_bhw)), _p(mask), int(mask_per_sample), _p(_f32c(w)), out.ptr(), out.ld,
         _p(stats), B, H, W, Cout, out.dt, _stream())


def conv3x3_c1_fwd_tiles(x_bhw, w, out, tiles, max_tiles, mask=None, mask_per_sample=False, want_stats=True):
    B, H, W = x_bhw.shape
    Cout = w.shape[0]
    assert out.C == Cout and (out.B, out.H, out.W) == (B, H, W) and (tiles.tile_h, tiles.tile_w) == (16, 16)
    stats = None
    if want_stats:
        stats = torch.empty((_lib.lib().cmu_conv3x3_c1_fwd_tiles_rows(int(max_tiles)), 2, Cout), dtype=torch.float32, device=out.buf.device)
    call("cmu_conv3x3_c1_fwd_tiles", _p(_f32c(x_bhw)), _p(mask), int(mask_per_sample), _p(_f32c(w)), out.ptr(), out.ld, _p(stats),
         _p(tiles.list), _p(tiles.count), int(max_tiles), B, H, W, Cout, out.dt, _stream())
    return stats


def conv3x3_c1_wgrad_bn_tiles(x_bhw, dA, yraw, scale, shift, save_mean, save_invstd, coef, dW, ws, tiles, max_tiles, mask=None,
                              mask_per_sample=False, w=None):
    B, H, W = x_bhw.shape
    assert (tiles.tile_h, tiles.tile_w) == (16, 16)
    call("cmu_conv3x3_c1_wgrad_bn_tiles", _p(_f32c(x_bhw)), _p(mask), int(mask_per_sample), dA.ptr(), dA.ld,
         None if w is not None else yraw.ptr(), 0 if w is not None else yraw.ld, None if w is None else _p(_f32c(w)), _p(scale), _p(shift),
         _p(save_mean), _p(save_invstd), _p(coef), _p(tiles.list), _p(tiles.count), int(max_tiles), _p(_f32c(dW)), B, H, W, dW.shape[0], dA.dt,
         _p(ws), _stream())


def conv3x3_fwd(x, wpacked, out, stats=None):
    assert x.dt == out.dt and (x.B, x.H, x.W) == (out.B, out.H, out.W)
    call("cmu_conv3x3_fwd", x.ptr(), x.ld, _p(x.scale), _p(x.shift), x.relu_from, _p(wpacked), out.ptr(), out.ld,
         _p(stats), x.B, x.H, x.W, x.C, out.C, x.dt, _stream(), work=2.0 * 9 * x.C * out.C * x.B * x.H * x.W)


def bn_finalize(stats, count, conv_bias, gamma, beta, running_mean, running_var, momentum, eps, training,
                scale, shift, save_mean, save_invstd, ws):
    C = scale.numel()
    nt = 0 if stats is None else stats.shape[0]
    need = _lib.lib().cmu_bn_finalize_ws_bytes(C)
    assert ws is None or ws.numel() * ws.element_size() >= need
    call("cmu_bn_finalize", _p(stats), nt, int(count), _p(conv_bias), _p(gamma), _p(beta), _p(running_mean),
         _p(running_var), float(momentum), float(eps), int(training), _p(scale), _p(shift), _p(save_mean),
         _p(save_invstd), C, _p(ws), _stream())


def bnrelu_maxpool_fwd(y, out):
    assert y.scale is not None
    call("cmu_bnrelu_maxpool_fwd", y.ptr(), y.ld, _p(y.scale), _p(y.shift), out.ptr(), out.ld, y.B, y.H, y.W, y.C,
         y.dt, _stream())


def convT2x2_fwd(x, wpacked, bias, out):
    Cout = out.C
    assert (out.H, out.W) == (2 * x.H, 2 * x.W)
    call("cmu_convT2x2_fwd", x.ptr(), x.ld, _p(x.scale), _p(x.shift), x.relu_from, _p(wpacked), _p(_f32c(bias)),
         out.ptr(), out.ld, x.B, x.H, x.W, x.C, Cout, x.dt, _stream(), work=2.0 * 4 * x.C * Cout * x.B * x.H * x.W)


def conv1x1_head_fwd(x, w, bias, logits):
    K = w.shape[0]
    call("cmu_conv1x1_head_fwd", x.ptr(), x.ld, _p(x.scale), _p(x.shift), _p(_f32c(w)), _p(_f32c(bias)),
         _p(_f32c(logits)), x.B, x.H, x.W, x.C, K, x.dt, _stream())


def apply_to_nchw(y, out=None):
    if out is None:
        out = torch.empty((y.B, y.C, y.H, y.W), dtype=torch.float32, device=y.buf.device)
    call("cmu_apply_to_nchw", y.ptr(), y.ld, _p(y.scale), _p(y.shift), y.relu_from, _p(out), y.B, y.H, y.W, y.C,
         y.dt, _stream())
    return out


def nchw_to_nhwc(x_nchw, out):
    B, C, H, W = x_nchw.shape
    call("cmu_nchw_to_nhwc", _p(_f32c(x_nchw)), out.ptr(), out.ld, B, H, W, C, out.dt, _stream())


def bn_bwd_reduce(dA, y, save_mean, save_invstd, dgamma, dbeta, coef, ws):
    call("cmu_bn_bwd_reduce", dA.ptr(), dA.ld, y.ptr(), y.ld, _p(y.scale), _p(y.shift), _p(save_mean), _p(save_invstd),
         _p(dgamma), _p(dbeta), _p(coef), y.B, y.H, y.W, y.C, y.dt, _p(ws), _stream())


def bn_bwd_apply(dA, y, save_mean, save_invstd, coef, dY):
    call("cmu_bn_bwd_apply", dA.ptr(), dA.ld, y.ptr(), y.ld, _p(y.scale), _p(y.shift), _p(save_mean), _p(save_invstd),
         _p(coef), dY.ptr(), dY.ld, y.B, y.H, y.W, y.C, y.dt, _stream())


def conv3x3_wgrad(x, dY, dW, ws):
    Cout, Cin = dW.shape[0], dW.shape[1]
    assert x.C == Cin and dY.C == Cout
    call("cmu_conv3x3_wgrad", x.ptr(), x.ld, _p(x.scale), _p(x.shift), x.relu_from, dY.ptr(), dY.ld, _p(_f32c(dW)),
         x.B, x.H, x.W, Cin, Cout, x.dt, _p(ws), _stream(), work=2.0 * 9 * Cin * Cout * x.B * x.H * x.W)


def conv3x3_c1_wgrad(x_bhw, dY, dW, ws, mask=None, mask_per_sample=False):
    B, H, W = x_bhw.shape
    call("cmu_conv3x3_c1_wgrad", _p(_f32c(x_bhw)), _p(mask), int(mask_per_sample), dY.ptr(), dY.ld, _p(_f32c(dW)),
         B, H, W, dW.shape[0], dY.dt, _p(ws), _stream())


def conv3x3_c1_wgrad_bn(x_bhw, dA, yraw, scale, shift, save_mean, save_invstd, coef, dW, ws, mask=None, mask_per_sample=False, w=None):
    B, H, W = x_bhw.shape
    assert dA.dt == yraw.dt
    if w is not None:
        call("cmu_conv3x3_c1_wgrad_bn_w", _p(_f32c(x_bhw)), _p(mask), int(mask_per_sample), dA.ptr(), dA.ld, _p(_f32c(w)), _p(scale), _p(shift),
             _p(save_mean), _p(save_invstd), _p(coef), _p(_f32c(dW)), B, H, W, dW.shape[0], dA.dt, _p(ws), _stream())
        return
    call("cmu_conv3x3_c1_wgrad_bn", _p(_f32c(x_bhw)), _p(mask), int(mask_per_sample), dA.ptr(), dA.ld, yraw.ptr(), yraw.ld,
         _p(scale), _p(shift), _p(save_mean), _p(save_invstd), _p(coef), _p(_f32c(dW)), B, H, W, dW.shape[0], dA.dt, _p(ws),
         _stream())


def maxpool_bwd(dP, dSkip, y, dA, save_mean=None, save_invstd=None, bn_ws=None, dSkip2=None):
    call("cmu_maxpool_bwd2", dP.ptr(), dP.ld, None if dSkip is None else dSkip.ptr(), 0 if dSkip is None else dSkip.ld,
         None if dSkip2 is None else dSkip2.ptr(), 0 if dSkip2 is None else dSkip2.ld, y.ptr(), y.ld, _p(y.scale), _p(y.shift),
         None if dA is None else dA.ptr(), 0 if dA is None else dA.ld, _p(save_mean), _p(save_invstd), _p(bn_ws),
         y.B, y.H, y.W, y.C, y.dt, _stream())


def maxpool_bwd_apply(dP, dSkip, y, save_mean, save_invstd, coef, dY, dSkip2=None):
    call("cmu_maxpool_bwd_apply", dP.ptr(), dP.ld, None if dSkip is None else dSkip.ptr(), 0 if dSkip is None else dSkip.ld,
         None if dSkip2 is None else dSkip2.ptr(), 0 if dSkip2 is None else dSkip2.ld, y.ptr(), y.ld, _p(y.scale), _p(y.shift),
         _p(save_mean), _p(save_invstd), _p(_f32c(coef)), dY.ptr(), dY.ld, y.B, y.H, y.W, y.C, y.dt, _stream())


def bn_bwd_finalize(bn_ws, count, dgamma, dbeta, coef):
    call("cmu_bn_bwd_finalize", _p(bn_ws), int(count), _p(dgamma), _p(dbeta), _p(coef), coef.shape[1], _stream())


def bn_bwd_finalize_tiles(bstats, count, dgamma, dbeta, coef, ws):
    call("cmu_bn_bwd_finalize_tiles", _p(bstats), bstats.shape[0], int(count), _p(dgamma), _p(dbeta), _p(coef), coef.shape[1], _p(ws),
         _stream())


def conv3x3_dgrad_bn(dY, wpacked_flip, dX, y, save_mean, save_invstd, bstats):
    call("cmu_conv3x3_dgrad_bn", dY.ptr(), dY.ld, _p(wpacked_flip), dX.ptr(), dX.ld, y.ptr(), y.ld, _p(y.scale), _p(y.shift),
         _p(save_mean), _p(save_invstd), _p(bstats), dX.B, dX.H, dX.W, dY.C, dX.C, dX.dt, _stream(),
         work=2.0 * 9 * dY.C * dX.C * dX.B * dX.H * dX.W)


def convT2x2_dgrad_bn(dOut, wpacked_dgrad, dX, y, save_mean, save_invstd, bstats):
    call("cmu_convT2x2_dgrad_bn", dOut.ptr(), dOut.ld, _p(wpacked_dgrad), dX.ptr(), dX.ld, y.ptr(), y.ld, _p(y.scale), _p(y.shift),
         _p(save_mean), _p(save_invstd), _p(bstats), dX.B, dX.H, dX.W, dX.C, dOut.C, dX.dt, _stream(),
         work=2.0 * 4 * dX.C * dOut.C * dX.B * dX.H * dX.W)


def convT2x2_dgrad(dOut, wpacked_dgrad, dX):
    call("cmu_convT2x2_dgrad", dOut.ptr(), dOut.ld, _p(wpacked_dgrad), dX.ptr(), dX.ld, dX.B, dX.H, dX.W, dX.C, dOut.C,
         dX.dt, _stream(), work=2.0 * 4 * dX.C * dOut.C * dX.B * dX.H * dX.W)


def convT2x2_wgrad(x, dOut, dW, dbias, ws):
    Cin, Cout = dW.shape[0], dW.shape[1]
    call("cmu_convT2x2_wgrad", x.ptr(), x.ld, _p(x.scale), _p(x.shift), x.relu_from, dOut.ptr(), dOut.ld, _p(_f32c(dW)),
         _p(_f32c(dbias)), x.B, x.H, x.W, Cin, Cout, x.dt, _p(ws), _stream(), work=2.0 * 4 * Cin * Cout * x.B * x.H * x.W)


def conv1x1_head_bn_apply(dlogits, x, w, save_mean, save_invstd, coef, dY):
    K = w.shape[0]
    call("cmu_conv1x1_head_bn_apply", _p(_f32c(dlogits)), x.ptr(), x.ld, _p(x.scale), _p(x.shift), _p(_f32c(w)), _p(save_mean),
         _p(save_invstd), _p(_f32c(coef)), dY.ptr(), dY.ld, x.B, x.H, x.W, x.C, K, x.dt, _stream())


def conv1x1_head_bwd(dlogits, x, w, dX, dW, dbias, ws, save_mean=None, save_invstd=None, bn_ws=None):
    K = w.shape[0]
    if dX is None:
        call("cmu_conv1x1_head_bwd", _p(_f32c(dlogits)), x.ptr(), x.ld, _p(x.scale), _p(x.shift), _p(_f32c(w)), None, 0,
             _p(_f32c(dW)), _p(_f32c(dbias)), _p(save_mean), _p(save_invstd), _p(bn_ws), x.B, x.H, x.W, x.C, K, x.dt, _p(ws),
             _stream())
        return
    call("cmu_conv1x1_head_bwd", _p(_f32c(dlogits)), x.ptr(), x.ld, _p(x.scale), _p(x.shift), _p(_f32c(w)), dX.ptr(), dX.ld,
         _p(_f32c(dW)), _p(_f32c(dbias)), _p(save_mean), _p(save_invstd), _p(bn_ws), x.B, x.H, x.W, x.C, K, x.dt, _p(ws),
         _stream())


def masked_mse_fwd_bwd(logits, channel, img, mask, loss, dlogits, loss_scale, ws, amp=None):
    B, K, H, W = logits.shape
    call("cmu_masked_mse_fwd_bwd", _p(_f32c(logits)), K, channel, _p(_f32c(img)), _p(mask), _p(loss), _p(dlogits),
         float(loss_scale), _p(None if amp is None else amp.state), B, H, W, _p(ws), _stream())


def softmax_ce_dice_fwd_bwd(logits, y1h, out, dlogits, loss_scale, ws):
    B, K, H, W = logits.shape
    assert K == 2 and y1h.dtype == torch.float64 and y1h.is_contiguous()
    call("cmu_softmax_ce_dice_fwd_bwd", _p(_f32c(logits)), _p(y1h), _p(out), _p(dlogits), float(loss_scale), B, H, W,
         _p(ws), _stream())


SEG_MAX_K = 8


def _seg_args(logits, y, class_w):
    B, K, H, W = logits.shape
    assert 2 <= K <= SEG_MAX_K and y.shape == logits.shape and y.is_contiguous() and y.dtype in (torch.float32, torch.float64)
    assert class_w is None or (class_w.shape == (K,) and class_w.dtype == torch.float32 and class_w.is_contiguous())
    return B, K, H, W


def seg_stats_fwd(logits, y, class_w, threshold, table, ws):
    B, K, H, W = _seg_args(logits, y, class_w)
    assert table.dtype == torch.float64 and table.numel() == 1 + 5 * K and table.is_contiguous()
    call("cmu_seg_stats_fwd", _p(_f32c(logits)), _p(y), int(y.dtype == torch.float64), _p(class_w), float(threshold), _p(table),
         B, K, H, W, _p(ws), _stream())


def seg_stats_bwd(logits, y, class_w, g_ce, g_tp, g_spr, dlogits):
    B, K, H, W = _seg_args(logits, y, class_w)
    for g, n in ((g_ce, 1), (g_tp, K), (g_spr, K)):
        assert g is None or (g.dtype == torch.float64 and g.numel() == n and g.is_contiguous())
    call("cmu_seg_stats_bwd", _p(_f32c(logits)), _p(y), int(y.dtype == torch.float64), _p(class_w), _p(g_ce), _p(g_tp), _p(g_spr),
         _p(_f32c(dlogits)), B, K, H, W, _stream())


PWL_KINDS = {"l1": 0, "mse": 1, "bce": 2, "bce_with_logits": 3}
PWL_MAX_C = 8


def _pwl_args(kind, x, y, chan_w, chan_pw):
    assert kind in PWL_KINDS, kind
    assert y.shape == x.shape and y.is_cuda and y.is_contiguous() and y.dtype in (torch.float32, torch.float64)
# ... 646 lines not shown
```

### include/cmunet_hip.h

```cpp
#ifndef CMUNET_HIP_H
#define CMUNET_HIP_H

#include <stdint.h>

#ifdef __cplusplus
extern "C" {
#endif

typedef enum { CMU_F32 = 0, CMU_F16 = 1, CMU_BF16 = 2 } cmu_dtype;

#define CMU_OK 0
#define CMU_ERR_ARG (-1)
#define CMU_ERR_UNSUPPORTED (-2)
#define CMU_ERR_WORKSPACE (-3)
#define CMU_ERR_LAUNCH (-4)

const char* cmu_last_error(void);
const char* cmu_last_kernel(void);
int cmu_version(void);
int cmu_set_dispatch_override(const char* name, int value);
const char* cmu_dispatch_knob_name(int index);
int cmu_get_dispatch_knob(const char* name, int* value, int* dflt);
int cmu_dtype_size(int dt);

int64_t cmu_pack_conv3x3_elems(int Cin, int Cout, int dt, int transpose_flip);
int cmu_pack_conv3x3(const float* w, void* out, int Cin, int Cout, int dt, int transpose_flip, void* stream);
int64_t cmu_pack_convT2x2_elems(int Cin, int Cout, int dt, int mode);
int cmu_pack_convT2x2(const float* w, void* out, int Cin, int Cout, int dt, int mode, void* stream);
int cmu_pack_desc_bytes(void);
int64_t cmu_pack_desc_blocks(int kind, int Cin, int Cout, int dt, int mode);
int cmu_pack_batch(const void* descs_dev, int ndesc, int64_t total_blocks, int dt, void* stream);

int cmu_conv3x3_c1_fwd(const float* x, const uint8_t* mask, int mask_per_sample, const float* w ,
                       void* y, int64_t ldy, float* stats, int B, int H, int W, int Cout, int dt, void* stream);

int cmu_conv3x3_fwd(const void* x, int64_t ldx, const float* in_scale, const float* in_shift, int relu_from,
                    const void* wpacked, void* y, int64_t ldy, float* stats,
                    int B, int H, int W, int Cin, int Cout, int dt, void* stream);
int cmu_conv_ntiles(int B, int H, int W);

int64_t cmu_bn_finalize_ws_bytes(int C);
int cmu_bn_finalize(const float* stats, int ntiles, int64_t count, const float* conv_bias, const float* gamma,
                    const float* beta, float* running_mean, float* running_var, float momentum, float eps,
                    int training, float* scale, float* shift, float* save_mean, float* save_invstd,
                    int C, void* ws, void* stream);

int cmu_bnrelu_maxpool_fwd(const void* y, int64_t ldy, const float* scale, const float* shift,
                           void* out, int64_t ldo, int B, int H, int W, int C, int dt, void* stream);

int cmu_convT2x2_fwd(const void* x, int64_t ldx, const float* in_scale, const float* in_shift, int relu_from,
                     const void* wpacked, const float* bias, void* out, int64_t ldo,
                     int B, int H, int W, int Cin, int Cout, int dt, void* stream);

int cmu_conv1x1_head_fwd(const void* x, int64_t ldx, const float* in_scale, const float* in_shift,
                         const float* w , const float* bias, float* logits,
                         int B, int H, int W, int C, int K, int dt, void* stream);

int cmu_apply_to_nchw(const void* y, int64_t ldy, const float* scale, const float* shift, int relu_from,
                      float* out, int B, int H, int W, int C, int dt, void* stream);
int cmu_nchw_to_nhwc(const float* x, void* out, int64_t ldo, int B, int H, int W, int C, int dt, void* stream);
int cmu_nhwc_to_nchw(const void* x, int64_t ldx, float* out, int B, int H, int W, int C, int dt, void* stream);

int64_t cmu_bn_bwd_ws_bytes(int C);
int cmu_bn_bwd_reduce(const void* dA, int64_t ldd, const void* y, int64_t ldy, const float* scale, const float* shift,
                      const float* save_mean, const float* save_invstd, float* dgamma, float* dbeta, float* coef,
                      int B, int H, int W, int C, int dt, void* ws, void* stream);
int cmu_bn_bwd_finalize(const void* bn_ws, int64_t count, float* dgamma, float* dbeta, float* coef, int C, void* stream);
int cmu_bn_bwd_finalize_tiles(const float* bstats, int ntiles, int64_t count, float* dgamma, float* dbeta, float* coef, int C,
                              void* ws, void* stream);
int cmu_conv3x3_dgrad_bn(const void* dY, int64_t ldd, const void* wpacked_flip, void* dX, int64_t ldx, const void* yraw, int64_t ldy,
                         const float* scale, const float* shift, const float* save_mean, const float* save_invstd, float* bstats,
                         int B, int H, int W, int K, int N, int dt, void* stream);
int cmu_bn_bwd_apply(const void* dA, int64_t ldd, const void* y, int64_t ldy, const float* scale, const float* shift,
                     const float* save_mean, const float* save_invstd, const float* coef, void* dY, int64_t ldo,
                     int B, int H, int W, int C, int dt, void* stream);

int64_t cmu_conv3x3_wgrad_ws_bytes(int B, int H, int W, int Cin, int Cout, int dt);
int cmu_conv3x3_wgrad(const void* x, int64_t ldx, const float* in_scale, const float* in_shift, int relu_from,
                      const void* dY, int64_t ldd, float* dW, int B, int H, int W, int Cin, int Cout, int dt,
                      void* ws, void* stream);
int64_t cmu_conv3x3_c1_wgrad_ws_bytes(int B, int H, int W, int Cout);
int cmu_conv3x3_c1_wgrad(const float* x, const uint8_t* mask, int mask_per_sample, const void* dY, int64_t ldd,
                         float* dW, int B, int H, int W, int Cout, int dt, void* ws, void* stream);
int cmu_conv3x3_c1_wgrad_bn(const float* x, const uint8_t* mask, int mask_per_sample, const void* dA, int64_t ldd,
                            const void* yraw, int64_t ldy, const float* scale, const float* shift, const float* save_mean,
                            const float* save_invstd, const float* coef, float* dW, int B, int H, int W, int Cout, int dt,
                            void* ws, void* stream);
int cmu_conv3x3_c1_wgrad_bn_w(const float* x, const uint8_t* mask, int mask_per_sample, const void* dA, int64_t ldd,
                              const float* w, const float* scale, const float* shift, const float* save_mean,
                              const float* save_invstd, const float* coef, float* dW, int B, int H, int W, int Cout, int dt,
                              void* ws, void* stream);

int cmu_maxpool_bwd(const void* dP, int64_t ldp, const void* dSkip, int64_t lds, const void* y, int64_t ldy,
                    const float* scale, const float* shift, void* dA, int64_t lda,
                    const float* save_mean, const float* save_invstd, void* bn_ws,
                    int B, int H, int W, int C, int dt, void* stream);
int cmu_maxpool_bwd2(const void* dP, int64_t ldp, const void* dSkip, int64_t lds, const void* dSkip2, int64_t lds2, const void* y,
                     int64_t ldy, const float* scale, const float* shift, void* dA, int64_t lda,
                     const float* save_mean, const float* save_invstd, void* bn_ws,
                     int B, int H, int W, int C, int dt, void* stream);
int cmu_maxpool_bwd_apply(const void* dP, int64_t ldp, const void* dSkip, int64_t lds, const void* dSkip2, int64_t lds2, const void* y,
                          int64_t ldy, const float* scale, const float* shift, const float* save_mean, const float* save_invstd,
                          const float* coef, void* dY, int64_t ldo, int B, int H, int W, int C, int dt, void* stream);

int cmu_bnrelu_maxpool_fwd_masked(const void* y, int64_t ldy, const float* scale, const float* shift, const uint8_t* active, int f,
                                  void* out, int64_t ldo, int B, int H, int W, int C, int dt, void* stream);
int cmu_maxpool_bwd_masked(const void* dP, int64_t ldp, const void* dSkip, int64_t lds, const void* y, int64_t ldy, const float* scale,
                           const float* shift, const uint8_t* active, int f, void* dA, int64_t lda, int B, int H, int W, int C, int dt,
                           void* stream);

int cmu_convT2x2_dgrad(const void* dOut, int64_t ldd, const void* wpacked_dgrad, void* dX, int64_t ldx,
                       int B, int H, int W, int Cin, int Cout, int dt, void* stream);
int cmu_convT2x2_dgrad_bn(const void* dOut, int64_t ldd, const void* wpacked_dgrad, void* dX, int64_t ldx, const void* yraw,
                          int64_t ldy, const float* scale, const float* shift, const float* save_mean, const float* save_invstd,
                          float* bstats, int B, int H, int W, int Cin, int Cout, int dt, void* stream);
int64_t cmu_convT2x2_wgrad_ws_bytes(int B, int H, int W, int Cin, int Cout, int dt);
int cmu_convT2x2_wgrad(const void* x, int64_t ldx, const float* in_scale, const float* in_shift, int relu_from,
                       const void* dOut, int64_t ldd, float* dW, float* dbias,
                       int B, int H, int W, int Cin, int Cout, int dt, void* ws, void* stream);

int64_t cmu_conv1x1_head_bwd_ws_bytes(int B, int H, int W, int C, int K);
int cmu_conv1x1_head_bwd(const float* dlogits, const void* x, int64_t ldx, const float* in_scale, const float* in_shift,
                         const float* w, void* dX, int64_t ldo, float* dW, float* dbias,
                         const float* save_mean, const float* save_invstd, void* bn_ws ,
                         int B, int H, int W, int C, int K, int dt, void* ws, void* stream);
int cmu_conv1x1_head_bn_apply(const float* dlogits, const void* x, int64_t ldx, const float* in_scale, const float* in_shift,
                              const float* w, const float* save_mean, const float* save_invstd, const float* coef, void* dY,
                              int64_t ldo, int B, int H, int W, int C, int K, int dt, void* stream);

int64_t cmu_masked_mse_ws_bytes(int B, int H);
int cmu_masked_mse_fwd_bwd(const float* logits, int K, int channel, const float* img, const uint8_t* mask,
                           float* loss, float* dlogits, float loss_scale, const void* amp_state, int B, int H, int W, void* ws,
                           void* stream);

int64_t cmu_softmax_ce_dice_ws_bytes(int B, int H, int W);
int cmu_softmax_ce_dice_fwd_bwd(const float* logits, const double* y1h, float* out, float* dlogits, float loss_scale,
                                int B, int H, int W, void* ws, void* stream);

int64_t cmu_seg_stats_ws_bytes(int K);
int cmu_seg_stats_fwd(const float* logits, const void* y, int y_is_f64, const float* class_w, float threshold, double* table,
                      int B, int K, int H, int W, void* ws, void* stream);
int cmu_seg_stats_bwd(const float* logits, const void* y, int y_is_f64, const float* class_w, const double* g_ce,
                      const double* g_tp, const double* g_spr, float* dlogits, int B, int K, int H, int W, void* stream);

#define CMU_PWL_L1 0
#define CMU_PWL_MSE 1
#define CMU_PWL_BCE 2
#define CMU_PWL_BCE_WITH_LOGITS 3
#define CMU_PWL_MAX_C 8
int64_t cmu_pointwise_loss_ws_bytes(void);
int cmu_pointwise_loss_fwd(int kind, const float* x, const void* y, int y_is_f64, const float* chan_w, const float* chan_pw,
                           double* out, int64_t outer, int C, int64_t inner, void* ws, void* stream);
int cmu_pointwise_loss_bwd(int kind, const float* x, const void* y, int y_is_f64, const float* chan_w, const float* chan_pw,
                           const double* g, float* dx, int64_t outer, int C, int64_t inner, void* stream);

// ... 261 lines not shown
```

Measured before the change: 845.0 images/sec.

## Fold encoder skip BN-backward stats into decoder and bottleneck dgrad epilogues

Adds a range-restricted conv3x3 dgrad-with-BN-stats entry point so the decoder concat dgrad and the next encoder dgrad can accumulate batch-norm backward partial sums for only a slice of channels (the skip part). A new forward pool kernel saves the raw pre-BN value that won each maxpool window. The encoder backward can then reuse these precomputed per-tile stats instead of running a separate maxpool-backward reduction pass over the full-resolution skip activation. The cost is an extra raw-pool tensor write in the forward pass, more branching in the igemm epilogue, and a fallback from the persistent kernel to the non-persistent one whenever a channel range is used.

```diff
diff --git a/cmunet_amd/_lib.py b/cmunet_amd/_lib.py
--- a/cmunet_amd/_lib.py
+++ b/cmunet_amd/_lib.py
@@ -79,6 +79,7 @@
     "cmu_bn_finalize_ws_bytes": (_L, [_I]),
     "cmu_bn_finalize": (_I, [_P, _I, _L, _P, _P, _P, _P, _P, _F, _F, _I, _P, _P, _P, _P, _I, _P, _P]),
     "cmu_bnrelu_maxpool_fwd": (_I, [_P, _L, _P, _P, _P, _L, _I, _I, _I, _I, _I, _P]),
+    "cmu_bnrelu_maxpool_fwd_raw": (_I, [_P, _L, _P, _P, _P, _L, _P, _L, _I, _I, _I, _I, _I, _P]),
     "cmu_convT2x2_fwd": (_I, [_P, _L, _P, _P, _I, _P, _P, _P, _L, _I, _I, _I, _I, _I, _I, _P]),
     "cmu_conv1x1_head_fwd": (_I, [_P, _L, _P, _P, _P, _P, _P, _I, _I, _I, _I, _I, _I, _P]),
     "cmu_apply_to_nchw": (_I, [_P, _L, _P, _P, _I, _P, _I, _I, _I, _I, _I, _P]),
@@ -100,6 +101,7 @@
     "cmu_convT2x2_dgrad": (_I, [_P, _L, _P, _P, _L, _I, _I, _I, _I, _I, _I, _P]),
     "cmu_convT2x2_dgrad_bn": (_I, [_P, _L, _P, _P, _L, _P, _L, _P, _P, _P, _P, _P, _I, _I, _I, _I, _I, _I, _P]),
     "cmu_conv3x3_dgrad_bn": (_I, [_P, _L, _P, _P, _L, _P, _L, _P, _P, _P, _P, _P, _I, _I, _I, _I, _I, _I, _P]),
+    "cmu_conv3x3_dgrad_bn_range": (_I, [_P, _L, _P, _P, _L, _P, _L, _P, _P, _P, _P, _P, _I, _I, _I, _I, _I, _I, _I, _I, _P]),
     "cmu_bn_bwd_finalize_tiles": (_I, [_P, _I, _L, _P, _P, _P, _I, _P, _P]),
     "cmu_convT2x2_wgrad_ws_bytes": (_L, [_I, _I, _I, _I, _I, _I]),
     "cmu_convT2x2_wgrad": (_I, [_P, _L, _P, _P, _I, _P, _L, _P, _P, _I, _I, _I, _I, _I, _I, _P, _P]),
@@ -210,7 +212,10 @@
 
 
 class CmuError(RuntimeError):
-    pass
+    rc = 0
+
+
+ERR_UNSUPPORTED = -2
 
 
 def build(verbose=False):
@@ -337,5 +342,7 @@
     else:
         rc = fn(*args)
     if rc != 0:
-        raise CmuError(f"{name} failed ({rc}): {l.cmu_last_error().decode()}")
+        err = CmuError(f"{name} failed ({rc}): {l.cmu_last_error().decode()}")
+        err.rc = rc
+        raise err
     return rc
diff --git a/cmunet_amd/csrc/conv_igemm.hip b/cmunet_amd/csrc/conv_igemm.hip
--- a/cmunet_amd/csrc/conv_igemm.hip
+++ b/cmunet_amd/csrc/conv_igemm.hip
@@ -31,6 +31,7 @@
     unsigned fd_nblk[2], fd_tx[2], fd_ty[2];
     const int* tile_list;
     const int* tile_count;
+    int bst_c0, bst_cs;
 };
 static inline void cmu_fastdiv_init(unsigned d, unsigned* out) {
     unsigned s = 0;
@@ -361,16 +362,18 @@
     }
     constexpr int CPRp = C::BN / C::EPC;
     u32x4 xr[CPRp];
-    if ((MODE != MODE_CONVT_FWD) && p.bstats != nullptr) {
+    const int bst_hi = p.bst_c0 + p.bst_cs;
+    const bool bs = (MODE != MODE_CONVT_FWD) && p.bstats != nullptr && n0 + C::BN > p.bst_c0 && n0 < bst_hi;
+    const int nq = n0 + (lane % CPRp) * C::EPC;
+    const bool bs_lane = bs && nq >= p.bst_c0 && nq < bst_hi;
+    if (bs_lane) {
 #pragma unroll
         for (int it = 0; it < CPRp; ++it) {
             const int idx = it * 64 + lane;
-            const int m = idx / CPRp, q = idx % CPRp;
+            const int m = idx / CPRp;
             const int row = 4 * wave + 2 * (m >> 5) + pm_row(m & 31), col = pm_col(m & 31);
             const int gy = ty0 + row < p.H ? ty0 + row : p.H - 1, gx = tx0 + col < p.W ? tx0 + col : p.W - 1;
-            int n = n0 + q * C::EPC;
-            n = n < p.N ? n : 0;
-            const int64_t xo = (((int64_t)b * p.H + gy) * p.W + gx) * p.ldbx + n;
+            const int64_t xo = (((int64_t)b * p.H + gy) * p.W + gx) * p.ldbx + (nq - p.bst_c0);
             xr[it] = ld_global16(reinterpret_cast<const unsigned char*>(p.bx) + xo * (int64_t)sizeof(elem_t));
         }
     }
@@ -407,14 +410,12 @@
     }
     constexpr int CPR = C::BN / C::EPC;
     unsigned char* yb = reinterpret_cast<unsigned char*>(p.y);
-    const bool bs = (MODE != MODE_CONVT_FWD) && p.bstats != nullptr;
     constexpr int EPCc = C::EPC;
     float bsc[EPCc], bsh[EPCc], bmu[EPCc], bis[EPCc], bs1[EPCc], bs2[EPCc];
-    const int nq = n0 + (lane % CPR) * EPCc;
     if (bs) {
 #pragma unroll
         for (int e = 0; e < EPCc; ++e) {
-            const int c = nq + e < p.N ? nq + e : 0;
+            const int c = bs_lane ? nq - p.bst_c0 + e : 0;
             bsc[e] = p.b_scale[c]; bsh[e] = p.b_shift[c]; bmu[e] = p.b_mean[c]; bis[e] = p.b_invstd[c];
             bs1[e] = bs2[e] = 0.f;
         }
@@ -436,7 +437,7 @@
                 off = (((int64_t)b * p.H + gy) * p.W + gx) * p.ldy + n;
             }
             st_global16(yb + off * (int64_t)sizeof(elem_t), v);
-            if (bs) {
+            if (bs_lane) {
                 float gv[EPCc], xv[EPCc];
                 TR::unpack(v, gv);
                 TR::unpack(xr[it], xv);
@@ -464,15 +465,15 @@
             }
         }
         __syncthreads();
-        if (tid < C::BN && n0 + tid < p.N) {
+        if (tid < C::BN && n0 + tid >= p.bst_c0 && n0 + tid < bst_hi) {
             float a = 0.f, q = 0.f;
 #pragma unroll
             for (int w4 = 0; w4 < 4; ++w4) {
                 a += stat_lds[(w4 * C::BN + tid) * 2 + 0];
                 q += stat_lds[(w4 * C::BN + tid) * 2 + 1];
             }
-            p.bstats[(tile * 2 + 0) * p.N + n0 + tid] = a;
-            p.bstats[(tile * 2 + 1) * p.N + n0 + tid] = q;
+            p.bstats[(tile * 2 + 0) * p.bst_cs + n0 + tid - p.bst_c0] = a;
+            p.bstats[(tile * 2 + 1) * p.bst_cs + n0 + tid - p.bst_c0] = q;
         }
     }
 }
@@ -896,6 +897,31 @@
     p.x = dY; p.ldx = ldd; p.w = wpacked_flip; p.y = dX; p.ldy = ldx;
     p.B = B; p.H = H; p.W = W; p.K = K; p.N = N; p.Cq = N;
     p.bx = yraw; p.ldbx = ldy; p.b_scale = scale; p.b_shift = shift; p.b_mean = save_mean; p.b_invstd = save_invstd; p.bstats = bstats;
+    p.bst_c0 = 0; p.bst_cs = N;
+    fill_tiles(p);
+    CMU_DISPATCH_DT(dt, conv3x3_fwd_t, p, (hipStream_t)stream);
+}
+
+extern "C" int cmu_conv3x3_dgrad_bn_range(const void* dY, int64_t ldd, const void* wpacked_flip, void* dX, int64_t ldx, const void* yraw,
+                                          int64_t ldy, const float* scale, const float* shift, const float* save_mean,
+                                          const float* save_invstd, float* bstats, int B, int H, int W, int K, int N, int c0, int Cs, int dt,
+                                          void* stream) {
+    CMU_CHECK_ARG(B > 0 && H > 0 && W > 0 && K > 0 && N > 0, "cmu_conv3x3_dgrad_bn_range: bad dims");
+    CMU_CHECK_ARG(cmu_dtype_size(dt) > 0, "cmu_conv3x3_dgrad_bn_range: bad dtype %d", dt);
+    const int epc = 16 / cmu_dtype_size(dt);
+    CMU_CHECK_ARG(c0 >= 0 && Cs > 0 && c0 + Cs <= N && c0 % epc == 0 && Cs % epc == 0,
+                  "cmu_conv3x3_dgrad_bn_range: channel range [%d, %d) must lie in [0, %d) in whole chunks of %d", c0, c0 + Cs, N, epc);
+    int rc;
+    if ((rc = check_act("cmu_conv3x3_dgrad_bn_range(dY)", dY, ldd, K, dt))) return rc;
+    if ((rc = check_act("cmu_conv3x3_dgrad_bn_range(dX)", dX, ldx, N, dt))) return rc;
+    if ((rc = check_bnstats("cmu_conv3x3_dgrad_bn_range(yraw)", yraw, ldy, scale, shift, save_mean, save_invstd, bstats, Cs, dt))) return rc;
+    CMU_CHECK_ARG(wpacked_flip && cmu_aligned16(wpacked_flip), "cmu_conv3x3_dgrad_bn_range: packed weights null/unaligned");
+    CMU_CHECK_ARG((int64_t)B * cmu_div_up(H, CMU_TH) * cmu_div_up(W, CMU_TW) * cmu_div_up(N, 64) < (1ll << 31), "cmu_conv3x3_dgrad_bn_range: grid too large");
+    IGParams p = {};
+    p.x = dY; p.ldx = ldd; p.w = wpacked_flip; p.y = dX; p.ldy = ldx;
+    p.B = B; p.H = H; p.W = W; p.K = K; p.N = N; p.Cq = N;
+    p.bx = yraw; p.ldbx = ldy; p.b_scale = scale; p.b_shift = shift; p.b_mean = save_mean; p.b_invstd = save_invstd; p.bstats = bstats;
+    p.bst_c0 = c0; p.bst_cs = Cs;
     fill_tiles(p);
     CMU_DISPATCH_DT(dt, conv3x3_fwd_t, p, (hipStream_t)stream);
 }
@@ -915,6 +941,7 @@
     p.x = dOut; p.ldx = ldd; p.w = wpacked_dgrad; p.y = dX; p.ldy = ldx;
     p.B = B; p.H = H; p.W = W; p.K = Cout; p.N = Cin; p.Cq = Cout;
     p.bx = yraw; p.ldbx = ldy; p.b_scale = scale; p.b_shift = shift; p.b_mean = save_mean; p.b_invstd = save_invstd; p.bstats = bstats;
+    p.bst_c0 = 0; p.bst_cs = Cin;
     fill_tiles(p);
     CMU_DISPATCH_DT(dt, convT_dgrad_t, p, (hipStream_t)stream);
 }
diff --git a/cmunet_amd/csrc/conv_igemm3.inc b/cmunet_amd/csrc/conv_igemm3.inc
--- a/cmunet_amd/csrc/conv_igemm3.inc
+++ b/cmunet_amd/csrc/conv_igemm3.inc
@@ -94,7 +94,8 @@
     }
 }
 template <int EPC>
-__device__ __forceinline__ void ig3_bst_fold(float (&bs1)[EPC], float (&bs2)[EPC], int lane, const float* mean, const float* invstd, float* stat) {
+__device__ __forceinline__ void ig3_bst_fold(float (&bs1)[EPC], float (&bs2)[EPC], int lane, const float* mean, const float* invstd, float* stat,
+                                             int lo = -(1 << 30), int hi = 1 << 30) {
     constexpr int H1 = EPC / 2, H2 = EPC / 4;
     float a1[H1], a2[H1], b1[H2], b2[H2];
     auto fold32 = [](float d, float s) {
@@ -111,7 +112,7 @@
 #pragma unroll
     for (int e = 0; e < H2; ++e) { b1[e] = fold8(fold16(a1[e], a1[e + H2])); b2[e] = fold8(fold16(a2[e], a2[e + H2])); }
     const int c0 = (lane & 7) * EPC + H1 * (lane >> 5) + H2 * ((lane >> 4) & 1);
-    if (!(lane & 8)) {
+    if (!(lane & 8) && c0 >= lo && c0 < hi) {
 #pragma unroll
         for (int e = 0; e < H2; ++e) {
             stat[(c0 + e) * 2 + 0] = b1[e];
@@ -150,11 +151,11 @@
     unsigned char* my = smem + wave * C::EPI_WAVE;
     unsigned char* yb = reinterpret_cast<unsigned char*>(p.y);
     constexpr int CPR = C::NFP * 32 / EPC;
-    auto write_slab = [&](float* dst) {
+    auto write_slab = [&](float* dst, int c_lo, int c_n) {
         if (tid < TWB * NB) {
             const int half = tid / NB, c = tid % NB;
             const int tx16 = TWB * tx + half, tiles16 = (p.W + 15) / 16;
-            if (tx16 < tiles16 && n0 + c < p.N) {
+            if (tx16 < tiles16 && n0 + c >= c_lo && n0 + c < c_lo + c_n) {
                 float a = 0.f, q = 0.f;
 #pragma unroll
                 for (int wr = 0; wr < C::RB; ++wr) {
@@ -163,11 +164,12 @@
                     q += stat_lds[(wv * 64 + (c & 63)) * 2 + 1];
                 }
                 const int64_t t16 = ((int64_t)b * p.tilesY + ty) * tiles16 + tx16;
-                dst[(t16 * 2 + 0) * p.N + n0 + c] = a;
-                dst[(t16 * 2 + 1) * p.N + n0 + c] = q;
-            }
-        }
-    };
+                dst[(t16 * 2 + 0) * c_n + n0 + c - c_lo] = a;
+                dst[(t16 * 2 + 1) * c_n + n0 + c - c_lo] = q;
+            }
+        }
+    };
+    const int bst_hi = p.bst_c0 + p.bst_cs;
     constexpr int NIT = (SW * 32 * CPR) / 64;
     float badd[2] = {0.f, 0.f};
     const bool cq64 = p.bias != nullptr && (p.Cq & 63) == 0;
@@ -183,16 +185,19 @@
     for (int jp = 0; jp < 2 / C::NFP; ++jp) {
         if (jp > 0) __syncthreads();
         u32x4 xr[NIT];
-        if (p.bstats != nullptr) {
+        const int nb0 = n0 + wn * 64 + jp * C::NFP * 32;
+        const int nq = nb0 + (lane % CPR) * EPC;
+        const bool bst_pass = p.bstats != nullptr && nb0 + C::NFP * 32 > p.bst_c0 && nb0 < bst_hi;
+        const bool bst_lane = bst_pass && nq >= p.bst_c0 && nq < bst_hi;
+        if (bst_lane) {
 #pragma unroll
             for (int it = 0; it < NIT; ++it) {
                 const int idx = it * 64 + lane;
-                const int m = idx / CPR, q = idx % CPR;
+                const int m = idx / CPR;
                 const int row = row0 + 2 * (m >> 5) + pm_row(m & 31), col = col0 + pm_col(m & 31);
                 const int gy = ty0 + row < p.H ? ty0 + row : p.H - 1, gx = tx0 + col < p.W ? tx0 + col : p.W - 1;
-                const int n = n0 + wn * 64 + jp * C::NFP * 32 + q * EPC;
                 const int64_t pixel = ((int64_t)b * p.H + gy) * p.W + gx;
-                xr[it] = ld_global16(reinterpret_cast<const unsigned char*>(p.bx) + (pixel * p.ldbx + n) * (int64_t)sizeof(elem_t));
+                xr[it] = ld_global16(reinterpret_cast<const unsigned char*>(p.bx) + (pixel * p.ldbx + nq - p.bst_c0) * (int64_t)sizeof(elem_t));
             }
         }
 #pragma unroll
@@ -206,11 +211,10 @@
                         TR::from_float(acc[i][jp * C::NFP + jj][e] + badd[jp * C::NFP + jj]);
                 }
         __syncthreads();
-        if (jp == 0 && p.stats != nullptr) write_slab(p.stats);
+        if (jp == 0 && p.stats != nullptr) write_slab(p.stats, 0, p.N);
         float bsc[EPC], bsh[EPC], bs1[EPC], bs2[EPC];
-        const int nq = n0 + wn * 64 + jp * C::NFP * 32 + (lane % CPR) * EPC;
-        if (p.bstats != nullptr) {
-            ig3_bst_consts<EPC>(p.b_scale, p.b_shift, nq, bsc, bsh);
+        if (bst_pass) {
+            ig3_bst_consts<EPC>(p.b_scale, p.b_shift, bst_lane ? nq - p.bst_c0 : 0, bsc, bsh);
 #pragma unroll
             for (int e = 0; e < EPC; ++e) bs1[e] = bs2[e] = 0.f;
         }
@@ -231,17 +235,16 @@
                 } else {
                     st_global16_nt(yb + (pixel * p.ldy + n) * (int64_t)sizeof(elem_t), v);
                 }
-                if (p.bstats != nullptr) ig3_bst_accum<TR>(v, xr[it], bsc, bsh, bs1, bs2);
-            }
-        }
-        if (p.bstats != nullptr) {
-            const int nb0 = n0 + wn * 64 + jp * C::NFP * 32;
-            ig3_bst_fold<EPC>(bs1, bs2, lane, p.b_mean + nb0, p.b_invstd + nb0, stat_lds + (wave * 64 + jp * C::NFP * 32) * 2);
-        }
+                if (bst_lane) ig3_bst_accum<TR>(v, xr[it], bsc, bsh, bs1, bs2);
+            }
+        }
+        if (bst_pass)
+            ig3_bst_fold<EPC>(bs1, bs2, lane, p.b_mean + (nb0 - p.bst_c0), p.b_invstd + (nb0 - p.bst_c0), stat_lds + (wave * 64 + jp * C::NFP * 32) * 2,
+                              p.bst_c0 - nb0, bst_hi - nb0);
     }
     if (p.bstats != nullptr) {
         __syncthreads();
-        write_slab(p.bstats);
+        write_slab(p.bstats, p.bst_c0, p.bst_cs);
     }
 }
 
diff --git a/cmunet_amd/csrc/conv_igemm3p.inc b/cmunet_amd/csrc/conv_igemm3p.inc
--- a/cmunet_amd/csrc/conv_igemm3p.inc
+++ b/cmunet_amd/csrc/conv_igemm3p.inc
@@ -589,6 +589,7 @@
 template <class TR>
 static int launch_igemm3_any(const IGParams& p, hipStream_t st) {
     if (!cmu_conv_persist_enabled()) return launch_igemm3<TR>(p, st);
+    if (p.bstats != nullptr && (p.bst_c0 != 0 || p.bst_cs != p.N)) return launch_igemm3<TR>(p, st);
     if (igemm6_eligible<TR>(p)) return launch_igemm6<TR>(p, st);
     if (igemm5_eligible<TR>(p)) return launch_igemm5<TR>(p, st);
     const bool tf = p.in_scale != nullptr, bst = p.bstats != nullptr;
diff --git a/cmunet_amd/csrc/elementwise.hip b/cmunet_amd/csrc/elementwise.hip
--- a/cmunet_amd/csrc/elementwise.hip
+++ b/cmunet_amd/csrc/elementwise.hip
@@ -633,6 +633,72 @@
     CMU_CHECK_ARG(cmu_aligned16(y) && cmu_aligned16(out), "cmu_bnrelu_maxpool_fwd: pointer alignment");
     CMU_DISPATCH_DT(dt, bnrelu_maxpool_t, y, ldy, scale, shift, out, ldo, B, H, W, C, (hipStream_t)stream);
 }
+template <class TR>
+__global__ void bnrelu_maxpool_raw_kernel(const unsigned char* __restrict__ y, int64_t ldy, const float* __restrict__ scale,
+                                          const float* __restrict__ shift, unsigned char* __restrict__ out, int64_t ldo,
+                                          unsigned char* __restrict__ raw, int64_t ldr, int B, int H, int W, int C, int64_t total) {
+    constexpr int EPC = TR::EPC;
+    constexpr int ES = (int)sizeof(typename TR::elem_t);
+    const int nchunk = C / EPC;
+    const int Ho = H / 2, Wo = W / 2;
+    for (int64_t o = (int64_t)blockIdx.x * blockDim.x + threadIdx.x; o < total; o += (int64_t)gridDim.x * blockDim.x) {
+        int ch, xo, yo, b;
+        int64_t pix;
+        if (total <= 0x7fffffffll) {
+            const unsigned ou = (unsigned)o, pq = ou / (unsigned)nchunk;
+            ch = (int)(ou - pq * (unsigned)nchunk);
+            pix = pq;
+        } else {
+            ch = (int)(o % nchunk);
+            pix = o / nchunk;
+        }
+        cmu_pixel_coords(pix, Wo, Ho, total <= 0x7fffffffll, b, yo, xo);
+        float sc[EPC], sh[EPC], m[EPC], best[EPC], win[EPC];
+#pragma unroll
+        for (int e = 0; e < EPC; ++e) {
+            sc[e] = scale[ch * EPC + e];
+            sh[e] = shift[ch * EPC + e];
+            m[e] = 0.f;
+        }
+#pragma unroll
+        for (int q = 0; q < 4; ++q) {
+            const int64_t src = (((int64_t)b * H + 2 * yo + (q >> 1)) * W + 2 * xo + (q & 1)) * ldy + ch * EPC;
+            float f[EPC];
+            TR::unpack(ld_global16_nt(y + src * ES), f);
+#pragma unroll
+            for (int e = 0; e < EPC; ++e) {
+                const float t = fmaf(f[e], sc[e], sh[e]);
+                m[e] = fmaxf(m[e], t);
+                const float a = fmaxf(t, 0.f);
+                if (q == 0 || a > best[e]) { best[e] = a; win[e] = f[e]; }
+            }
+        }
+        const int64_t dst = (((int64_t)b * Ho + yo) * Wo + xo);
+        st_global16(out + (dst * ldo + ch * EPC) * ES, TR::pack(m));
+        st_global16(raw + (dst * ldr + ch * EPC) * ES, TR::pack(win));
+    }
+}
+template <class TR>
+static int bnrelu_maxpool_raw_t(const void* y, int64_t ldy, const float* scale, const float* shift, void* out, int64_t ldo, void* raw,
+                                int64_t ldr, int B, int H, int W, int C, hipStream_t st) {
+    const int64_t total = (int64_t)B * (H / 2) * (W / 2) * (C / TR::EPC);
+    const int grid = (int)(cmu_div_up64(total, 256) < CMU_POOLF_CAP ? cmu_div_up64(total, 256) : CMU_POOLF_CAP);
+    hipLaunchKernelGGL((bnrelu_maxpool_raw_kernel<TR>), dim3(grid), dim3(256), 0, st, (const unsigned char*)y, ldy, scale, shift,
+                       (unsigned char*)out, ldo, (unsigned char*)raw, ldr, B, H, W, C, total);
+    CMU_CHECK_LAUNCH("cmu_bnrelu_maxpool_fwd_raw");
+    return CMU_OK;
+}
+extern "C" int cmu_bnrelu_maxpool_fwd_raw(const void* y, int64_t ldy, const float* scale, const float* shift, void* out, int64_t ldo,
+                                          void* raw, int64_t ldr, int B, int H, int W, int C, int dt, void* stream) {
+    const int es = cmu_dtype_size(dt);
+    CMU_CHECK_ARG(es > 0 && y && out && raw && scale && shift, "cmu_bnrelu_maxpool_fwd_raw: bad args");
+    const int epc = 16 / es;
+    CMU_CHECK_ARG(H % 2 == 0 && W % 2 == 0 && H > 0 && W > 0 && B > 0, "cmu_bnrelu_maxpool_fwd_raw: H,W must be even (got %d,%d)", H, W);
+    CMU_CHECK_ARG(C % epc == 0 && ldy % epc == 0 && ldo % epc == 0 && ldr % epc == 0 && ldy >= C && ldo >= C && ldr >= C,
+                  "cmu_bnrelu_maxpool_fwd_raw: C/ld alignment");
+    CMU_CHECK_ARG(cmu_aligned16(y) && cmu_aligned16(out) && cmu_aligned16(raw), "cmu_bnrelu_maxpool_fwd_raw: pointer alignment");
+    CMU_DISPATCH_DT(dt, bnrelu_maxpool_raw_t, y, ldy, scale, shift, out, ldo, raw, ldr, B, H, W, C, (hipStream_t)stream);
+}
 extern "C" int cmu_bnrelu_maxpool_fwd_masked(const void* y, int64_t ldy, const float* scale, const float* shift, const uint8_t* active, int f,
                                              void* out, int64_t ldo, int B, int H, int W, int C, int dt, void* stream) {
     const int es = cmu_dtype_size(dt);
diff --git a/cmunet_amd/engine.py b/cmunet_amd/engine.py
--- a/cmunet_amd/engine.py
+++ b/cmunet_amd/engine.py
@@ -16,6 +16,7 @@
 _FUSE_POOL = os.environ.get("CMU_POOL_FUSE", "1") != "0"
 _POISON_NEW = os.environ.get("CMU_POISON_NEW", "0") == "1"
 _FUSE_POOL2 = os.environ.get("CMU_POOL_FUSE2", "1") != "0"
+_POOL_SUMS = os.environ.get("CMU_POOL_SUMS", "0") == "1"
 _C1W_RECOMP = os.environ.get("CMU_C1W_RECOMP", "1") != "0"
 
 
@@ -169,7 +170,7 @@
         n = ops.ntiles(y.B, y.H, y.W)
         return self.scratch.get("bst", n * 2 * y.C * 4)[:n * 2 * y.C * 4].view(torch.float32).view(n, 2, y.C)
 
-    def _convbn_bwd(self, sd, s, dA, grads, need_dx, dx_out=None, fused_stats=False, next_bn=None, head=None, pool=None):
+    def _convbn_bwd(self, sd, s, dA, grads, need_dx, dx_out=None, fused_stats=False, next_bn=None, head=None, pool=None, share=None):
         y = s["y"]
         B, H, W, C = y.B, y.H, y.W, y.C
         w = sd[s["pconv"] + "weight"]
@@ -217,6 +218,18 @@
         if not need_dx or first:
             return None
         dX = dx_out if dx_out is not None else self._new(B, H, W, w.shape[1])
+        if share is not None:
+            sy, smean, sinvstd, rows, c0, plan, key = share
+            try:
+                if c0 == 0 and sy.C == dX.C:
+                    ops.conv3x3_dgrad_bn(dY, self._wp(s["pconv"], w, True), dX, sy, smean, sinvstd, rows)
+                else:
+                    ops.conv3x3_dgrad_bn_range(dY, self._wp(s["pconv"], w, True), dX, sy, smean, sinvstd, rows, c0)
+                plan[key] = True
+                return dX
+            except _lib.CmuError as e:
+                if e.rc != _lib.ERR_UNSUPPORTED:
+                    raise
         if next_bn is not None and next_bn["y"].C == dX.C and (_FUSE_DGRAD_BN == "1" or (_FUSE_DGRAD_BN == "64" and dX.C <= 64)
                                                                 or (_FUSE_DGRAD_BN == "128" and dX.C <= 128)):
             slab = self._tile_slab(next_bn["y"])
@@ -233,7 +246,8 @@
             n += 1
         return n
 
-    def encoder_forward(self, sd, x_bhw, training, prefix="", mask=None, mask_per_sample=False, skip_out=None, skip_affine=None):
+    def encoder_forward(self, sd, x_bhw, training, prefix="", mask=None, mask_per_sample=False, skip_out=None, skip_affine=None,
+                        pool_raw=False):
         B, H, W = x_bhw.shape
         nd = self.n_down(sd, prefix)
         assert H % (1 << nd) == 0 and W % (1 << nd) == 0, f"H,W must be multiples of {1 << nd}"
@@ -248,8 +262,13 @@
             s1, s2 = self._double_conv_fwd(sd, p, x_act, out2, training, x_img, mask if i == 1 else None, mask_per_sample,
                                            affine_out2=skip_affine[i - 1] if skip_affine is not None else None)
             pooled = self._new(B, h // 2, w_ // 2, C)
-            ops.bnrelu_maxpool_fwd(s2["y"], pooled)
-            ctx["levels"].append({"s1": s1, "s2": s2, "pooled": pooled})
+            lvl = {"s1": s1, "s2": s2, "pooled": pooled}
+            if pool_raw and training and _POOL_SUMS:
+                lvl["raw"] = self._new(B, h // 2, w_ // 2, C)
+                ops.bnrelu_maxpool_fwd_raw(s2["y"], pooled, lvl["raw"])
+            else:
+                ops.bnrelu_maxpool_fwd(s2["y"], pooled)
+            ctx["levels"].append(lvl)
             x_act, x_img = pooled, None
             h, w_ = h // 2, w_ // 2
         p = f"{prefix}double_conv.double_conv."
@@ -262,10 +281,34 @@
         self.flush_counters()
         return ctx
 
-    def encoder_backward(self, sd, ctx, d_latent, d_skips, grads, after_bottleneck=None):
+    def _pool_sums_plan(self, ectx, dctx):
+        plan = []
+        for i, lv in enumerate(ectx["levels"]):
+            ent = None
+            dl = dctx["levels"][i] if i < len(dctx["levels"]) else None
+            if _POOL_SUMS and "raw" in lv and dl is not None:
+                y2, cat = lv["s2"]["y"], dl["cat"]
+                sf = bool(cat.get("skip_first", False))
+                if y2.buf is cat["buf"] and y2.coff == cat.get("base", 0) + (0 if sf else cat["Cup"]) and y2.C == cat["Cskip"]:
+                    nf, nh = ops.ntiles(y2.B, y2.H, y2.W), ops.ntiles(y2.B, y2.H // 2, y2.W // 2)
+                    nb = (nf + nh) * 2 * y2.C * 4
+                    slab = self.scratch.get(("pool_sums", i), nb)[:nb].view(torch.float32).view(nf + nh, 2, y2.C)
+                    ent = {"slab": slab, "nf": nf, "skip": False, "pool": False}
+            plan.append(ent)
+        return plan
+
+    def encoder_backward(self, sd, ctx, d_latent, d_skips, grads, after_bottleneck=None, pool_sums=None):
         b = ctx["bott"]
         dA = self._convbn_bwd(sd, b["s2"], d_latent, grads, True, next_bn=b["s1"])
-        dP = self._convbn_bwd(sd, b["s1"], dA, grads, len(ctx["levels"]) > 0)
+        def pooled_share(i):
+            ent = pool_sums[i - 1] if (pool_sums is not None and i >= 1) else None
+            if ent is None or not ent["skip"]:
+                return None
+            lv = ctx["levels"][i - 1]
+            y2 = lv["s2"]["y"]
+            return (lv["raw"].with_transform(y2.scale, y2.shift, 0), lv["s2"]["mean"], lv["s2"]["invstd"], ent["slab"][ent["nf"]:], 0, ent, "pool")
+
+        dP = self._convbn_bwd(sd, b["s1"], dA, grads, len(ctx["levels"]) > 0, share=pooled_share(len(ctx["levels"])))
         if after_bottleneck is not None:
             self.flush_zero_bias()
             after_bottleneck()
@@ -274,14 +317,18 @@
             y2 = lv["s2"]["y"]
             ds = d_skips[i - 1] if d_skips is not None else None
             ds, ds2 = ds if isinstance(ds, (tuple, list)) else (ds, None)
-            if _FUSE_POOL and (ds2 is None or _FUSE_POOL2):
+            ent = pool_sums[i - 1] if pool_sums is not None else None
+            if ent is not None and ent["skip"] and ent["pool"] and ds2 is None and _FUSE_POOL:
+                lv["s2"]["bstats"] = ent["slab"]
+                dA1 = self._convbn_bwd(sd, lv["s2"], None, grads, True, fused_stats=True, next_bn=lv["s1"], pool=(dP, ds, None))
+            elif _FUSE_POOL and (ds2 is None or _FUSE_POOL2):
                 ops.maxpool_bwd(dP, ds, y2, None, lv["s2"]["mean"], lv["s2"]["invstd"], self._bn_ws(y2.C), dSkip2=ds2)
                 dA1 = self._convbn_bwd(sd, lv["s2"], None, grads, True, fused_stats=True, next_bn=lv["s1"], pool=(dP, ds, ds2))
             else:
                 dA2 = self._new(y2.B, y2.H, y2.W, y2.C)
                 ops.maxpool_bwd(dP, ds, y2, dA2, lv["s2"]["mean"], lv["s2"]["invstd"], self._bn_ws(y2.C), dSkip2=ds2)
                 dA1 = self._convbn_bwd(sd, lv["s2"], dA2, grads, True, fused_stats=True, next_bn=lv["s1"])
-            dP = self._convbn_bwd(sd, lv["s1"], dA1, grads, i > 1)
+            dP = self._convbn_bwd(sd, lv["s1"], dA1, grads, i > 1, share=pooled_share(i - 1))
         self.flush_zero_bias()
         return None
 
@@ -410,7 +457,7 @@
         self.flush_counters()
         return ctx
 
-    def decoder_backward(self, sd, ctx, dlogits, grads, need_input_grads=True, latent_bn=None):
+    def decoder_backward(self, sd, ctx, dlogits, grads, need_input_grads=True, latent_bn=None, pool_sums=None, enc_levels=None):
         prefix = ctx["prefix"]
         x = ctx["out"]
         K = sd[prefix + "conv_last.weight"].shape[0]
@@ -435,8 +482,13 @@
             Cup, Cs = cat["Cup"], cat["Cskip"]
             dA1 = self._convbn_bwd(sd, lv["s2"], dA, grads, True, fused_stats=(fused and i == 1), next_bn=lv["s1"],
                                    head=head if i == 1 else None)
-            dcat = self._convbn_bwd(sd, lv["s1"], dA1, grads, True)
             sf = bool(cat.get("skip_first", False))
+            share = None
+            ent = pool_sums[i - 1] if pool_sums is not None else None
+            if ent is not None:
+                e2 = enc_levels[i - 1]["s2"]
+                share = (e2["y"], e2["mean"], e2["invstd"], ent["slab"][:ent["nf"]], 0 if sf else Cup, ent, "skip")
+            dcat = self._convbn_bwd(sd, lv["s1"], dA1, grads, True, share=share)
             d_skips[i - 1] = Act(dcat.buf, 0 if sf else Cup, Cs)
             dleft = Act(dcat.buf, Cs if sf else 0, Cup)
             wt = sd[p + "up_sample.weight"]
@@ -476,7 +528,7 @@
             owns = True
         skip_out = [Act(c["buf"], c["Cup"], c["Cskip"]) for c in cats]
         skip_affine = [(c["scale"][c["Cup"]:], c["shift"][c["Cup"]:]) for c in cats]
-        ectx = self.encoder_forward(sd, x_bhw, training, "", mask, mask_per_sample, skip_out, skip_affine)
+        ectx = self.encoder_forward(sd, x_bhw, training, "", mask, mask_per_sample, skip_out, skip_affine, pool_raw=True)
         dctx = self.decoder_forward(sd, ectx["latent"], ectx["skips"], training, "", cats, True)
         ctx = _Ctx(enc=ectx, dec=dctx)
         if owns and training:
@@ -485,10 +537,12 @@
 
     def unet_backward(self, sd, ctx, dlogits, after_decoder=None, after_bottleneck=None):
         grads = {}
-        d_latent, d_skips = self.decoder_backward(sd, ctx["dec"], dlogits, grads, True, latent_bn=ctx["enc"]["bott"]["s2"])
+        plan = self._pool_sums_plan(ctx["enc"], ctx["dec"])
+        d_latent, d_skips = self.decoder_backward(sd, ctx["dec"], dlogits, grads, True, latent_bn=ctx["enc"]["bott"]["s2"],
+                                                  pool_sums=plan, enc_levels=ctx["enc"]["levels"])
         if after_decoder is not None:
             after_decoder()
-        self.encoder_backward(sd, ctx["enc"], d_latent, d_skips, grads, after_bottleneck)
+        self.encoder_backward(sd, ctx["enc"], d_latent, d_skips, grads, after_bottleneck, pool_sums=plan)
         if self._cats is not None and ctx["dec"]["cats"] is self._cats[1]:
             self._cats_busy = False
         return grads
diff --git a/cmunet_amd/ops.py b/cmunet_amd/ops.py
--- a/cmunet_amd/ops.py
+++ b/cmunet_amd/ops.py
@@ -215,6 +215,12 @@
          y.dt, _stream())
 
 
+def bnrelu_maxpool_fwd_raw(y, out, raw):
+    assert y.scale is not None and (raw.B, raw.H, raw.W, raw.C) == (out.B, out.H, out.W, out.C)
+    call("cmu_bnrelu_maxpool_fwd_raw", y.ptr(), y.ld, _p(y.scale), _p(y.shift), out.ptr(), out.ld, raw.ptr(), raw.ld, y.B, y.H, y.W, y.C,
+         y.dt, _stream())
+
+
 def convT2x2_fwd(x, wpacked, bias, out):
     Cout = out.C
     assert (out.H, out.W) == (2 * x.H, 2 * x.W)
@@ -301,6 +307,12 @@
 def conv3x3_dgrad_bn(dY, wpacked_flip, dX, y, save_mean, save_invstd, bstats):
     call("cmu_conv3x3_dgrad_bn", dY.ptr(), dY.ld, _p(wpacked_flip), dX.ptr(), dX.ld, y.ptr(), y.ld, _p(y.scale), _p(y.shift),
          _p(save_mean), _p(save_invstd), _p(bstats), dX.B, dX.H, dX.W, dY.C, dX.C, dX.dt, _stream(),
+         work=2.0 * 9 * dY.C * dX.C * dX.B * dX.H * dX.W)
+
+
+def conv3x3_dgrad_bn_range(dY, wpacked_flip, dX, y, save_mean, save_invstd, bstats, c0):
+    call("cmu_conv3x3_dgrad_bn_range", dY.ptr(), dY.ld, _p(wpacked_flip), dX.ptr(), dX.ld, y.ptr(), y.ld, _p(y.scale), _p(y.shift),
+         _p(save_mean), _p(save_invstd), _p(bstats), dX.B, dX.H, dX.W, dY.C, dX.C, int(c0), y.C, dX.dt, _stream(),
          work=2.0 * 9 * dY.C * dX.C * dX.B * dX.H * dX.W)
 
 
diff --git a/include/cmunet_hip.h b/include/cmunet_hip.h
--- a/include/cmunet_hip.h
+++ b/include/cmunet_hip.h
@@ -47,6 +47,8 @@
 
 int cmu_bnrelu_maxpool_fwd(const void* y, int64_t ldy, const float* scale, const float* shift,
                            void* out, int64_t ldo, int B, int H, int W, int C, int dt, void* stream);
+int cmu_bnrelu_maxpool_fwd_raw(const void* y, int64_t ldy, const float* scale, const float* shift, void* out, int64_t ldo,
+                               void* raw, int64_t ldr, int B, int H, int W, int C, int dt, void* stream);
 
 int cmu_convT2x2_fwd(const void* x, int64_t ldx, const float* in_scale, const float* in_shift, int relu_from,
                      const void* wpacked, const float* bias, void* out, int64_t ldo,
@@ -71,6 +73,9 @@
 int cmu_conv3x3_dgrad_bn(const void* dY, int64_t ldd, const void* wpacked_flip, void* dX, int64_t ldx, const void* yraw, int64_t ldy,
                          const float* scale, const float* shift, const float* save_mean, const float* save_invstd, float* bstats,
                          int B, int H, int W, int K, int N, int dt, void* stream);
+int cmu_conv3x3_dgrad_bn_range(const void* dY, int64_t ldd, const void* wpacked_flip, void* dX, int64_t ldx, const void* yraw, int64_t ldy,
+                               const float* scale, const float* shift, const float* save_mean, const float* save_invstd, float* bstats,
+                               int B, int H, int W, int K, int N, int c0, int Cs, int dt, void* stream);
 int cmu_bn_bwd_apply(const void* dA, int64_t ldd, const void* y, int64_t ldy, const float* scale, const float* shift,
                      const float* save_mean, const float* save_invstd, const float* coef, void* dY, int64_t ldo,
                      int B, int H, int W, int C, int dt, void* stream);
```

Measured after the change: 842.9 images/sec. No clear change (-0.3%).
